# elvinlife/RadioSaber

Measured on AMD Instinct MI355X. Metric: scheduled TTIs/sec (and us/TTI) at 20 slices x 500 UEs x 25 RBGs; HBM GB/s, higher is better.
Workload: dtype f64

## Files before the change

### include/radiosaber_hip.h

```cpp
#ifndef RADIOSABER_HIP_H_
#define RADIOSABER_HIP_H_

#include <stddef.h>
#include <stdint.h>

#ifdef __cplusplus
extern "C" {
#endif

#define RS_ABI_VERSION 11

enum {
  RS_OK = 0,
  RS_ERR_INVALID = -1,
  RS_ERR_NO_DEVICE = -2,
  RS_ERR_HIP = -3,
  RS_ERR_STATE = -4,
  RS_ERR_RANGE = -5
};

enum {
  RS_SCHED_PF = 1,
  RS_SCHED_NVS = 7,
  RS_SCHED_SEQUENTIAL = 8,
  RS_SCHED_MAXCELL = 9,
  RS_SCHED_NVS_NONGREEDY = 11,
  RS_SCHED_UPPERBOUND = 10,
  RS_SCHED_SUBOPT = 101,
  RS_SCHED_VOGEL = 103
};

#define RS_MAX_SLICES 64
#define RS_MAX_RBGS 64
#define RS_MAX_USERS 1024

typedef struct rs_config {
  int32_t n_slices;
  int32_t n_users;
  int32_t n_rbgs;
  int32_t rbg_size;
  int32_t sched;
  int32_t device;
  const double* slice_weight;
  const int32_t* algo_alpha;
  const int32_t* algo_beta;
  const int32_t* algo_epsilon;
  const int32_t* algo_psi;
  const int32_t* user_to_slice;
  void* stream;
  int32_t synthetic_exp;
  int32_t link_tables;
} rs_config;

enum { RS_LINK_DEFAULT = 0, RS_LINK_HOST_LIBM = 1, RS_LINK_PINNED_GLIBC_2_35 = 2 };

const char* rs_last_error(void);
int rs_abi_version(void);
int rs_device_count(void);

int rs_link_tables(double eff[16], double kbps[16], double eesm_e[16], double eesm_x[16]);
int rs_link_tables_pinned(double eff[16], double kbps[16], double eesm_e[16], double eesm_x[16]);
int rs_link_tables_compare(char* msg, size_t msglen);

int rs_get_rbg_size(int nb_rbs);
int rs_dl_prbs_for_bandwidth(double bw_mhz);

typedef struct rs_ctx rs_ctx;

rs_ctx* rs_create(const rs_config* cfg);
rs_ctx* rs_create_checked(const rs_config* cfg, int abi_version, size_t cfg_size);
#define RS_CREATE(cfg) rs_create_checked((cfg), RS_ABI_VERSION, sizeof(rs_config))
void rs_destroy(rs_ctx* ctx);

typedef struct rs_tti_in {
  int32_t n_users;
  const int32_t* user_id;
  const uint8_t* cqi;
  const double* avg_rate;
  int32_t rand0, rand1;
  const uint8_t* cqi_prb;
  const double* hol_delay;
  const uint8_t* prio_has_data;
  const int32_t* rand_draws;
  const int32_t* required_rbs;
  const int32_t* data_to_transmit;
  uint64_t cqi_epoch;
} rs_tti_in;

typedef struct rs_tti_out {
  int32_t* target_rbs;
  int32_t* quota_rbgs;
  int32_t* rbg_to_user;
  int32_t* user_nprb;
  int32_t* user_final_cqi;
  int32_t* user_mcs;
  int32_t* user_tbs_bits;
  int32_t* upper_rbg;
  int32_t* upper_user;
} rs_tti_out;

int rs_schedule_tti(rs_ctx* ctx, const rs_tti_in* in, rs_tti_out* out);
int rs_ctx_specialize(rs_ctx* ctx);
int rs_ctx_jit_status(rs_ctx* ctx, char* msg, size_t msglen);
int rs_jit_selfcheck_dropin(int n_slices, int n_users, int n_rbgs, int rbg_size, int threads, int sched, char* err, size_t errlen);
int rs_get_slice_offset(rs_ctx* ctx, double* offset );
int rs_set_slice_offset(rs_ctx* ctx, const double* offset );

#define RS_GROUP_MAX_CELLS 1024
typedef struct rs_group rs_group;
rs_group* rs_group_create(const rs_config* cfg, int32_t n_cells);
rs_group* rs_group_create_checked(const rs_config* cfg, int32_t n_cells, int abi_version, size_t cfg_size);
#define RS_GROUP_CREATE(cfg, n_cells) rs_group_create_checked((cfg), (n_cells), RS_ABI_VERSION, sizeof(rs_config))
void rs_group_destroy(rs_group* g);
int rs_group_schedule_tti(rs_group* g, int32_t n, const int32_t* cell_ids, const rs_tti_in* in , rs_tti_out* out );
int rs_group_get_slice_offset(rs_group* g, int32_t cell, double* offset );
// ... 163 lines not shown
```

### radiosaber_amd/__init__.py

```python
from . import toolchain as _toolchain

_toolchain.prefer_system_compiler()

from .api import (
    RS_SCHED_MAXCELL, RS_SCHED_NVS, RS_SCHED_PF, RS_SCHED_NVS_NONGREEDY, RS_SCHED_SEQUENTIAL, RS_SCHED_UPPERBOUND, RS_SCHED_VOGEL, RS_SCHED_SUBOPT,
    BEARER_BACKLOG, BEARER_NONE, BEARER_QUEUE, FULL_PACKET, TRACE_CQI_HISTOGRAM, frames_to_bursts, internet_flow_arrivals,
    BatchScheduler, GroupScheduler, RadioSaberError, SliceConfig, TtiResult, TtiScheduler, device_count, device_source_hash, dl_prbs_for_bandwidth, get_rbg_size, hbm_copy_probe, jit_selfcheck, lds_bytes_per_cell,
    jit_cache_file, jit_cache_stats, jit_cache_warm, jit_compiler_identity, lib, link_tables_compare,
    RS_LINK_DEFAULT, RS_LINK_HOST_LIBM, RS_LINK_PINNED_GLIBC_2_35,
    link_tables, load_trace_dir, read_trace_mapping, read_ue_trace,
)

__all__ = ["RS_SCHED_PF", "RS_SCHED_NVS", "RS_SCHED_SEQUENTIAL", "RS_SCHED_MAXCELL", "RS_SCHED_VOGEL", "RS_SCHED_SUBOPT", "RS_SCHED_UPPERBOUND", "RS_SCHED_NVS_NONGREEDY", "SliceConfig",
           "TtiScheduler", "GroupScheduler", "TtiResult", "BatchScheduler", "RadioSaberError", "device_count", "lib",
           "link_tables", "jit_selfcheck", "device_source_hash", "TRACE_CQI_HISTOGRAM", "read_trace_mapping", "read_ue_trace",
           "load_trace_dir", "hbm_copy_probe", "lds_bytes_per_cell", "get_rbg_size", "dl_prbs_for_bandwidth", "internet_flow_arrivals", "frames_to_bursts",
           "BEARER_NONE", "BEARER_BACKLOG", "BEARER_QUEUE", "FULL_PACKET", "jit_cache_file", "jit_cache_stats", "jit_cache_warm",
           "jit_compiler_identity", "link_tables_compare", "RS_LINK_DEFAULT", "RS_LINK_HOST_LIBM", "RS_LINK_PINNED_GLIBC_2_35"]
```

### radiosaber_amd/api.py

```python
import ctypes as C
import json
import os
from dataclasses import dataclass, field
from pathlib import Path
from typing import List, Optional, Sequence

import numpy as np

RS_SCHED_SUBOPT = 101
RS_SCHED_PF, RS_SCHED_NVS, RS_SCHED_SEQUENTIAL, RS_SCHED_MAXCELL, RS_SCHED_UPPERBOUND, RS_SCHED_NVS_NONGREEDY, RS_SCHED_VOGEL = \
    1, 7, 8, 9, 10, 11, 103

TRACE_CQI_HISTOGRAM = (152600, 56656, 270880, 2088792, 3509504, 1595568, 4145392, 5295816, 1903424,
                       6890232, 4770864, 2842552, 3579624, 96000, 1227696)

_PKG = Path(__file__).resolve().parent
_LIB_PATH = Path(os.environ.get("RS_HIP_LIB", _PKG / "libradiosaber_hip.so"))


class RadioSaberError(RuntimeError):
    def __init__(self, code, msg):
        super().__init__(f"radiosaber_hip error {code}: {msg}")
        self.code = code

# ... 15 lines not shown


RS_LINK_DEFAULT, RS_LINK_HOST_LIBM, RS_LINK_PINNED_GLIBC_2_35 = 0, 1, 2

RS_ABI_VERSION = 11


class _TtiIn(C.Structure):
    _fields_ = [("n_users", C.c_int32), ("user_id", C.POINTER(C.c_int32)),
                ("cqi", C.POINTER(C.c_uint8)), ("avg_rate", C.POINTER(C.c_double)),
                ("rand0", C.c_int32), ("rand1", C.c_int32), ("cqi_prb", C.POINTER(C.c_uint8)),
                ("hol_delay", C.POINTER(C.c_double)), ("prio_has_data", C.POINTER(C.c_uint8)),
                ("rand_draws", C.POINTER(C.c_int32)),
                ("required_rbs", C.POINTER(C.c_int32)), ("data_to_transmit", C.POINTER(C.c_int32)), ("cqi_epoch", C.c_uint64)]


class _TtiOut(C.Structure):
    _fields_ = [("target_rbs", C.POINTER(C.c_int32)), ("quota_rbgs", C.POINTER(C.c_int32)),
                ("rbg_to_user", C.POINTER(C.c_int32)), ("user_nprb", C.POINTER(C.c_int32)),
                ("user_final_cqi", C.POINTER(C.c_int32)), ("user_mcs", C.POINTER(C.c_int32)),
                ("user_tbs_bits", C.POINTER(C.c_int32)),
                ("upper_rbg", C.POINTER(C.c_int32)), ("upper_user", C.POINTER(C.c_int32))]


class _BatchLog(C.Structure):
    _fields_ = [("rbg_to_user", C.POINTER(C.c_int16)), ("tbs_bits", C.POINTER(C.c_int32)),
                ("quota", C.POINTER(C.c_int16)), ("target", C.POINTER(C.c_int16)), ("uinfo", C.POINTER(C.c_int32)),
                ("slice_keys", C.POINTER(C.c_uint32))]


class _BatchBearerLog(C.Structure):
    _fields_ = [("bytes", C.POINTER(C.c_int32)), ("hol_delay", C.POINTER(C.c_double))]


ABI_SYMBOLS = [
    "rs_last_error", "rs_abi_version", "rs_device_count", "rs_link_tables",
    "rs_create", "rs_destroy", "rs_schedule_tti", "rs_get_slice_offset", "rs_set_slice_offset",
    "rs_batch_create", "rs_batch_destroy", "rs_batch_seed", "rs_batch_upload_cqi_epochs",
    "rs_batch_synthesize_cqi", "rs_batch_download_cqi_epochs", "rs_batch_set_trace",
    "rs_batch_run", "rs_batch_run_async", "rs_batch_sync", "rs_batch_run_logged",
    "rs_batch_run_timed", "rs_batch_read_state", "rs_batch_slice_bytes_device",
    "rs_batch_slice_bytes", "rs_jit_selfcheck", "rs_jit_selfcheck_queue", "rs_batch_debug_stamps", "rs_batch_ttis_done", "rs_batch_stream", "rs_batch_kernel_name",
    "rs_trace_read_mapping", "rs_trace_read_ue_log", "rs_trace_load_dir", "rs_hbm_copy_probe", "rs_lds_bytes_per_cell",
    "rs_get_rbg_size", "rs_dl_prbs_for_bandwidth", "rs_batch_synthesize_cqi_at", "rs_batch_run_logged_ex",
    "rs_batch_read_clock", "rs_batch_jit_status", "rs_batch_prepare_launch",
    "rs_batch_upload_cqi_epochs_prb", "rs_batch_set_trace_prb",
    "rs_batch_set_bearers", "rs_batch_set_arrivals", "rs_batch_read_bearer_state", "rs_internet_flow_arrivals",
    "rs_device_source_hash",
    "rs_create_checked", "rs_batch_create_checked", "rs_jit_selfcheck_untuned", "rs_batch_write_state",
    "rs_ctx_specialize", "rs_jit_selfcheck_dropin",
    "rs_batch_debug_heap_sorts", "rs_ctx_debug_heap_sorts",
    "rs_jit_cache_stats", "rs_jit_cache_file", "rs_jit_cache_warm", "rs_batch_autotune_report", "rs_batch_debug_clocks",
    "rs_batch_checkpoint_bytes", "rs_batch_checkpoint_save", "rs_batch_checkpoint_load",
    "rs_link_tables_pinned", "rs_link_tables_compare", "rs_ctx_jit_status", "rs_jit_compiler_identity",
    "rs_batch_flow_record", "rs_batch_run_logged_bearers",
    "rs_group_create", "rs_group_create_checked", "rs_group_destroy", "rs_group_schedule_tti",
    "rs_group_get_slice_offset", "rs_group_set_slice_offset", "rs_group_launch_count", "rs_group_kernel_name",
    "rs_group_image_stats", "rs_group_specialize", "rs_group_jit_status", "rs_jit_selfcheck_group",
    "rs_group_set_avg", "rs_group_get_avg", "rs_group_set_pending", "rs_group_schedule_tti_at", "rs_group_run_at",
    "rs_group_specialize_resident", "rs_group_resident_jit_status", "rs_jit_selfcheck_group_resident",
    "rs_group_set_bearers", "rs_group_get_bearers", "rs_group_schedule_tti_queued",
    "rs_group_specialize_queued", "rs_group_queued_jit_status", "rs_jit_selfcheck_group_queued",
    "rs_group_set_counters", "rs_group_get_counters", "rs_group_schedule_tti_counted",
    "rs_group_set_flows", "rs_group_get_flows", "rs_group_schedule_tti_flows",
    "rs_group_specialize_counted", "rs_group_counted_jit_status", "rs_jit_selfcheck_group_counted",
    "rs_group_specialize_flows", "rs_group_flows_jit_status", "rs_jit_selfcheck_group_flows",
    "rs_group_specialize_run", "rs_group_run_jit_status", "rs_jit_selfcheck_group_run",
]

_lib = None


def lib():
    global _lib
    if _lib is not None:
        return _lib
    if not _LIB_PATH.exists():
        raise RadioSaberError(-100, f"{_LIB_PATH} is missing: run `python -m radiosaber_amd.build` "
                                    "(there is no CPU fallback)")
    L = C.CDLL(str(_LIB_PATH))
    L.rs_last_error.restype = C.c_char_p
    L.rs_link_tables.argtypes = [C.POINTER(C.c_double)] * 4
    L.rs_link_tables_pinned.argtypes = [C.POINTER(C.c_double)] * 4
    L.rs_link_tables_compare.argtypes = [C.c_char_p, C.c_size_t]
    L.rs_ctx_jit_status.argtypes = [C.c_void_p, C.c_char_p, C.c_size_t]
    L.rs_jit_compiler_identity.restype = C.c_char_p
    L.rs_jit_compiler_identity.argtypes = []
    L.rs_create.restype = C.c_void_p
    L.rs_create.argtypes = [C.POINTER(_Config)]
    L.rs_destroy.argtypes = [C.c_void_p]
    L.rs_schedule_tti.argtypes = [C.c_void_p, C.POINTER(_TtiIn), C.POINTER(_TtiOut)]
    L.rs_get_slice_offset.argtypes = [C.c_void_p, C.POINTER(C.c_double)]
    L.rs_set_slice_offset.argtypes = [C.c_void_p, C.POINTER(C.c_double)]
    L.rs_group_create.restype = C.c_void_p
    L.rs_group_create.argtypes = [C.POINTER(_Config), C.c_int32]
    L.rs_group_create_checked.restype = C.c_void_p
    L.rs_group_create_checked.argtypes = [C.POINTER(_Config), C.c_int32, C.c_int, C.c_size_t]
    L.rs_group_destroy.argtypes = [C.c_void_p]
    L.rs_group_schedule_tti.argtypes = [C.c_void_p, C.c_int32, C.POINTER(C.c_int32), C.POINTER(_TtiIn), C.POINTER(_TtiOut)]
    L.rs_group_get_slice_offset.argtypes = [C.c_void_p, C.c_int32, C.POINTER(C.c_double)]
    L.rs_group_set_slice_offset.argtypes = [C.c_void_p, C.c_int32, C.POINTER(C.c_double)]
    L.rs_group_launch_count.restype = C.c_int64
    L.rs_group_launch_count.argtypes = [C.c_void_p]
    L.rs_group_image_stats.argtypes = [C.c_void_p, C.POINTER(C.c_int64)]
    L.rs_group_kernel_name.restype = C.c_char_p
    L.rs_group_kernel_name.argtypes = [C.c_void_p]
    L.rs_group_specialize.argtypes = [C.c_void_p]
    L.rs_group_set_avg.argtypes = [C.c_void_p, C.c_int32, C.POINTER(C.c_double), C.c_double]
    L.rs_group_get_avg.argtypes = [C.c_void_p, C.c_int32, C.POINTER(C.c_double), C.POINTER(C.c_int32), C.POINTER(C.c_double)]
    L.rs_group_set_pending.argtypes = [C.c_void_p, C.c_int32, C.POINTER(C.c_int32)]
    L.rs_group_schedule_tti_at.argtypes = [C.c_void_p, C.c_int32, C.POINTER(C.c_int32), C.POINTER(_TtiIn), C.POINTER(_TtiOut), C.POINTER(C.c_double)]
    L.rs_group_run_at.argtypes = [C.c_void_p, C.c_int32, C.POINTER(C.c_int32), C.POINTER(_TtiIn), C.c_int32, C.POINTER(C.c_double),
                                  C.POINTER(C.c_int32), C.POINTER(_TtiOut)]
    L.rs_group_set_bearers.argtypes = [C.c_void_p, C.c_int32, C.POINTER(C.c_uint8), C.POINTER(C.c_double), C.c_double]
    L.rs_group_get_bearers.argtypes = [C.c_void_p, C.c_int32, C.POINTER(C.c_double), C.POINTER(C.c_int32), C.POINTER(C.c_double)]
    L.rs_group_schedule_tti_queued.argtypes = [C.c_void_p, C.c_int32, C.POINTER(C.c_int32), C.POINTER(_TtiIn), C.POINTER(_TtiOut),
                                               C.POINTER(C.c_double), C.POINTER(C.POINTER(C.c_int32))]
    L.rs_group_jit_status.argtypes = [C.c_void_p, C.c_char_p, C.c_size_t]
    L.rs_jit_selfcheck_group.argtypes = [C.c_int] * 6 + [C.c_char_p, C.c_size_t]
    L.rs_group_specialize_resident.argtypes = [C.c_void_p]
    L.rs_group_resident_jit_status.argtypes = [C.c_void_p, C.c_char_p, C.c_size_t]
    L.rs_jit_selfcheck_group_resident.argtypes = [C.c_int] * 6 + [C.c_char_p, C.c_size_t]
    L.rs_group_set_counters.argtypes = [C.c_void_p, C.c_int32, C.POINTER(C.c_int64), C.POINTER(C.c_int64)]
    L.rs_group_get_counters.argtypes = [C.c_void_p, C.c_int32, C.POINTER(C.c_int64), C.POINTER(C.c_int64)]
    L.rs_group_schedule_tti_counted.argtypes = [C.c_void_p, C.c_int32, C.POINTER(C.c_int32), C.POINTER(_TtiIn), C.POINTER(_TtiOut),
                                                C.POINTER(C.c_double), C.POINTER(C.POINTER(C.c_int32)), C.POINTER(C.POINTER(C.c_int32))]
    L.rs_group_set_flows.argtypes = [C.c_void_p, C.c_int32, C.POINTER(C.c_uint8), C.POINTER(C.c_double), C.c_double, C.POINTER(C.c_int64),
                                     C.POINTER(C.c_int64)]
    L.rs_group_get_flows.argtypes = [C.c_void_p, C.c_int32, C.POINTER(C.c_double), C.POINTER(C.c_int32), C.POINTER(C.c_double),
                                     C.POINTER(C.c_int64), C.POINTER(C.c_int64)]
    L.rs_group_schedule_tti_flows.argtypes = [C.c_void_p, C.c_int32, C.POINTER(C.c_int32), C.POINTER(_TtiIn), C.POINTER(_TtiOut),
                                              C.POINTER(C.c_double), C.POINTER(C.POINTER(C.c_uint8))]
    L.rs_group_specialize_queued.argtypes = [C.c_void_p]
    L.rs_group_queued_jit_status.argtypes = [C.c_void_p, C.c_char_p, C.c_size_t]
    L.rs_jit_selfcheck_group_queued.argtypes = [C.c_int] * 6 + [C.c_char_p, C.c_size_t]
    L.rs_group_specialize_counted.argtypes = [C.c_void_p]
# ... 102 lines not shown
                  group=False, resident=False, queued=False, counted=False, flows=False, run=False):
    _jit_flags(False, False, group, resident, queued, counted, flows, run)
    buf = C.create_string_buffer(4096)
    fn = lib().rs_jit_selfcheck_queue if queues else (lib().rs_jit_selfcheck_untuned if untuned else lib().rs_jit_selfcheck)
    if dropin:
        fn = lib().rs_jit_selfcheck_dropin
    if group:
        fn = lib().rs_jit_selfcheck_group_resident if resident else lib().rs_jit_selfcheck_group
        if queued:
            fn = lib().rs_jit_selfcheck_group_queued
        if counted:
            fn = lib().rs_jit_selfcheck_group_counted
        if flows:
            fn = lib().rs_jit_selfcheck_group_flows
        if run:
            fn = lib().rs_jit_selfcheck_group_run
    n = fn(n_slices, n_users, n_rbgs, rbg_size, threads, sched, buf, 4096)
    if n < 0:
        raise RadioSaberError(n, buf.value.decode(errors="replace"))
    return n


def jit_cache_stats():
    out = (C.c_longlong * 4)()
    lib().rs_jit_cache_stats(out)
    return dict(zip(("hits", "misses", "stores", "rejected"), (int(x) for x in out)))


def _jit_flags(lean, streamed, group, resident, queued=False, counted=False, flows=False, run=False):
    if run and not (group and resident):
        raise ValueError("run=True needs group=True and resident=True: the run kernel is the resident form's")
    if run and (queued or counted or flows):
        raise ValueError("run=True excludes queued=True, counted=True and flows=True: only the resident form has a run")
    if counted and not group:
        raise ValueError("counted=True needs group=True: only a group has a counted kernel")
    if flows and not group:
        raise ValueError("flows=True needs group=True: only a group has a flows kernel")
    if counted and resident:
        raise ValueError("resident=True and counted=True exclude each other: two forms of a group's kernel")
    if flows and (resident or queued or counted):
        raise ValueError("flows=True excludes resident=True, queued=True and counted=True: a form of a group's kernel of its own")
    if counted:
        queued = True
    if resident and not group:
        raise ValueError("resident=True needs group=True: only a group has a resident kernel")
    if queued and not group:
        raise ValueError("queued=True needs group=True: only a group has a queued kernel")
    if queued and resident:
        raise ValueError("resident=True and queued=True exclude each other: two forms of a group's kernel")
    return (4 if lean else 0) | (2 if streamed else 0) | (8 if group else 0) | (16 if resident else 0) | (32 if queued else 0) | \
        (64 if counted else 0) | (128 if flows else 0) | (256 if run else 0)


def jit_cache_file(n_slices, n_users, n_rbgs, rbg_size, threads=512, sched=RS_SCHED_MAXCELL, lean=False, streamed=False, group=False,
                   resident=False, queued=False, counted=False, flows=False, run=False):
    buf = C.create_string_buffer(4096)
    lib().rs_jit_cache_file(n_slices, n_users, n_rbgs, rbg_size, threads, sched, _jit_flags(lean, streamed, group, resident, queued, counted, flows, run),
                            buf, 4096)
    return buf.value.decode()


def jit_cache_warm(n_slices, n_users, n_rbgs, rbg_size, threads=512, sched=RS_SCHED_MAXCELL, lean=False, streamed=False, group=False,
                   resident=False, queued=False, counted=False, flows=False, run=False):
    buf = C.create_string_buffer(4096)
    n = lib().rs_jit_cache_warm(n_slices, n_users, n_rbgs, rbg_size, threads, sched, _jit_flags(lean, streamed, group, resident, queued, counted, flows, run),
                                buf, 4096)
    if n < 0:
        raise RadioSaberError(n, buf.value.decode(errors="replace"))
    return n


def device_count():
    return lib().rs_device_count()


def device_source_hash():
    return lib().rs_device_source_hash().decode()


def get_rbg_size(nb_rbs):
    return _count(lib().rs_get_rbg_size(nb_rbs))


def dl_prbs_for_bandwidth(bw_mhz):
    return lib().rs_dl_prbs_for_bandwidth(float(bw_mhz))


BEARER_NONE, BEARER_BACKLOG, BEARER_QUEUE = 0, 1, 2
FULL_PACKET = 1495


def internet_flow_arrivals(rate_mbps, start_time, stop_time, size_seed, max_bursts=1 << 16):
    t = np.zeros(max_bursts, np.float64)
    nf = np.zeros(max_bursts, np.int32)
    la = np.zeros(max_bursts, np.int32)
    n = _count(lib().rs_internet_flow_arrivals(rate_mbps, start_time, stop_time, size_seed, max_bursts, _p(t, C.c_double),
                                               _p(nf, C.c_int32), _p(la, C.c_int32)))
    return t[:n].copy(), nf[:n].copy(), la[:n].copy()


def frames_to_bursts(times, frame_bytes, mtu=1490):
    fb = np.asarray(frame_bytes, np.int64)
    rem = fb % mtu
    return (np.ascontiguousarray(times, np.float64), (fb // mtu).astype(np.int32),
            np.where(rem > 0, rem + (FULL_PACKET - mtu), 0).astype(np.int32))


def lds_bytes_per_cell(n_slices, n_users, n_rbgs, sched=RS_SCHED_MAXCELL, threads=512):
    return _count(lib().rs_lds_bytes_per_cell(n_slices, n_users, n_rbgs, sched, threads))


def hbm_copy_probe(device=0, nbytes=1 << 30, iters=10):
    g = C.c_double(0)
    _check(lib().rs_hbm_copy_probe(device, nbytes, iters, C.byref(g)))
    return g.value


def link_tables(pinned=False):
    out = [np.zeros(16, np.float64) for _ in range(4)]
    _check((lib().rs_link_tables_pinned if pinned else lib().rs_link_tables)(*[_p(a, C.c_double) for a in out]))
    return dict(zip(("eff", "kbps", "eesm_e", "eesm_x"), out))


def link_tables_compare():
    buf = C.create_string_buffer(4096)
    return _count(lib().rs_link_tables_compare(buf, 4096)), buf.value.decode(errors="replace")


def jit_compiler_identity():
    return lib().rs_jit_compiler_identity().decode()


def read_trace_mapping(path, max_entries=4096):
    out = np.zeros(max_entries, dtype=np.int32)
    n = _count(lib().rs_trace_read_mapping(os.fsencode(str(path)), _p(out, C.c_int32), max_entries))
    if n > max_entries:
        raise RadioSaberError(-1, f"{path}: {n} entries, max_entries={max_entries}")
    return out[:n].copy()


def read_ue_trace(path, nb_rbs=512, rbg_size=8, n_rows=475, per_prb=False):
    R = nb_rbs // rbg_size
    rbg = np.zeros((n_rows, R), dtype=np.uint8)
    prb = np.zeros((n_rows, nb_rbs), dtype=np.uint8) if per_prb else None
    rc = _count(lib().rs_trace_read_ue_log(os.fsencode(str(path)), n_rows, nb_rbs, rbg_size, _p(rbg, C.c_uint8),
                                           _p(prb, C.c_uint8) if per_prb else None))
    return (prb if per_prb else rbg), rc


def load_trace_dir(directory, n_traces=158, nb_rbs=512, rbg_size=8, n_rows=475):
    R = nb_rbs // rbg_size
    out = np.zeros((n_traces, n_rows, R), dtype=np.uint8)
    rc = _count(lib().rs_trace_load_dir(os.fsencode(str(directory)), n_traces, n_rows, nb_rbs, rbg_size,
                                        _p(out, C.c_uint8)))
    return out, rc


@dataclass
class SliceConfig:
    ues_per_slice: List[int]
    weight: List[float] = field(default_factory=list)
    algo_alpha: List[int] = field(default_factory=list)
    algo_beta: List[int] = field(default_factory=list)
    algo_epsilon: List[int] = field(default_factory=list)
    algo_psi: List[int] = field(default_factory=list)
    traffic: List[dict] = field(default_factory=list)

    def __post_init__(self):
        S = len(self.ues_per_slice)
        if not self.weight:
            self.weight = [1.0 / S] * S
        for name, default in (("algo_alpha", 0), ("algo_beta", 0), ("algo_epsilon", 1), ("algo_psi", 1)):
            if not getattr(self, name):
                setattr(self, name, [default] * S)
# ... 618 lines not shown
        _check(lib().rs_batch_set_arrivals(self._h, _p(off, C.c_int64), _p(t_all, C.c_double), _p(nf_all, C.c_int32),
                                           _p(la_all, C.c_int32)))
        self._burst_slots = {key: (int(off[(key[0] * self.U + key[1]) * 2 + key[2]]), len(v[0])) for key, v in bursts.items()}
        self._n_bursts = total

    def flow_record(self):
        if not hasattr(self, "_burst_slots"):
            raise RadioSaberError(-4, "flow_record() before set_arrivals()")
        tti = np.zeros(max(self._n_bursts, 1), np.int32)
        tm = np.zeros(max(self._n_bursts, 1), np.float64)
        _check(lib().rs_batch_flow_record(self._h, _p(tti, C.c_int32), _p(tm, C.c_double)))
        return {key: (tti[i:i + n].copy(), tm[i:i + n].copy()) for key, (i, n) in self._burst_slots.items()}

    def bearer_state(self):
        shp = (self.n_cells, self.U, 2)
        avg, cb, cr = np.zeros(shp, np.float64), np.zeros(shp, np.int64), np.zeros(shp, np.int64)
        qb, qp = np.zeros(shp, np.int32), np.zeros(shp, np.int32)
        _check(lib().rs_batch_read_bearer_state(self._h, _p(avg, C.c_double), _p(cb, C.c_int64), _p(cr, C.c_int64),
                                                _p(qb, C.c_int32), _p(qp, C.c_int32)))
        return {"avg_rate": avg, "cum_bytes": cb, "cum_rbs": cr, "queue_bytes": qb, "queue_packets": qp}

    def clock(self):
        t = np.zeros(self.n_cells, np.float64)
        lu = np.zeros(self.n_cells, np.float64)
        _check(lib().rs_batch_read_clock(self._h, _p(t, C.c_double), _p(lu, C.c_double)))
        return t, lu

    def prepare_launch(self, n_ttis):
        _check(lib().rs_batch_prepare_launch(self._h, int(n_ttis)))

    def checkpoint(self):
        n = _count(lib().rs_batch_checkpoint_bytes(self._h))
        buf = C.create_string_buffer(n)
        _check(lib().rs_batch_checkpoint_save(self._h, buf, n))
        return buf.raw

    def restore(self, blob):
        _check(lib().rs_batch_checkpoint_load(self._h, blob, len(blob)))

    def debug_clocks(self):
        mhz = np.zeros(self.n_cells, np.float64)
        ms = np.zeros(self.n_cells, np.float64)
        _check(lib().rs_batch_debug_clocks(self._h, _p(mhz, C.c_double), _p(ms, C.c_double)))
        return mhz, ms

    def autotune_report(self):
        buf = C.create_string_buffer(1024)
        n = lib().rs_batch_autotune_report(self._h, buf, 1024)
        return n, buf.value.decode(errors="replace")

    def jit_status(self):
        if not getattr(self, "_h", None):
            raise RadioSaberError(-4, "jit_status() of a closed batch")
        buf = C.create_string_buffer(512)
        rc = lib().rs_batch_jit_status(self._h, buf, 512)
        return rc, buf.value.decode(errors="replace")

    def slice_bytes(self):
        out = np.zeros(self.S, np.uint64)
        _check(lib().rs_batch_slice_bytes(self._h, _p(out, C.c_uint64)))
        return out

    def slice_bytes_into(self, device_ptr):
        _check(lib().rs_batch_slice_bytes_device(self._h, C.c_void_p(device_ptr)))

    def heap_sorts(self):
        out = np.zeros((self.n_cells, 3), np.int64)
        _check(lib().rs_batch_debug_heap_sorts(self._h, _p(out, C.c_int64)))
        return out

    def debug_stamps(self, cell=0):
        out = np.zeros(20, np.uint64)
        _check(lib().rs_batch_debug_stamps(self._h, cell, _p(out, C.c_uint64)))
        return out

    @property
    def ttis_done(self):
        return lib().rs_batch_ttis_done(self._h)

    @property
    def stream(self):
        return lib().rs_batch_stream(self._h)

    @property
    def kernel_name(self):
        return lib().rs_batch_kernel_name(self._h).decode()
```

### radiosaber_amd/csrc/rs_api.cpp

```cpp
#include <hip/hip_runtime_api.h>

#include <atomic>
#include <chrono>
#include <cmath>
#include <cstdarg>
#include <cstdio>
#include <cstdlib>
#include <cstring>
#include <new>
#include <random>
#include <fstream>
#include <vector>

#include "../../include/radiosaber_hip.h"
#include "rs_amc_tables.inc"
#include "rs_link_pinned.inc"
#include "rs_device.h"

extern "C" hipError_t rs_launch_cells(const RsLaunch* p, int threads, hipStream_t stream);
extern "C" hipError_t rs_prepare_kernels(int max_lds_bytes);
struct RsJitKernel;
extern "C" RsJitKernel* rs_jit_get(int device, int S, int U, int R, int G, int NT, int sched, int qmode, int win, char* err, size_t errlen,
                                   int flags,
                                   const char* variant = nullptr);
extern "C" int rs_jit_is_untuned(const RsJitKernel* k);
extern "C" int rs_jit_is_verified(const RsJitKernel* k);
extern "C" int rs_jit_was_loaded(const RsJitKernel* k);
extern "C" void rs_jit_mark_verified(RsJitKernel* k);
extern "C" void rs_jit_reject(RsJitKernel* k);
extern "C" hipError_t rs_jit_launch(RsJitKernel* k, const RsLaunch* p, hipStream_t stream);
extern "C" hipError_t rs_launch_synth(uint8_t* epochs, int64_t grid_stride, int n_cells, int n_epochs, int U, int R, int Upad,
                                      uint64_t seed, int64_t first_cell, const uint32_t* cdf16, hipStream_t stream);
extern "C" hipError_t rs_launch_copy_probe(const void* src, void* dst, size_t bytes, hipStream_t stream);
extern "C" hipError_t rs_launch_slice_bytes(const int64_t* cum_bytes, const uint8_t* user_slice, int n_cells, int U,
                                            int S, unsigned long long* d_out, hipStream_t stream);

namespace {

thread_local char g_err[512] = "";

int fail(int code, const char* fmt, ...) {
  va_list ap;
  va_start(ap, fmt);
  vsnprintf(g_err, sizeof g_err, fmt, ap);
  va_end(ap);
  return code;
}

#define HIP_TRY(expr)                                                                          \
  do {                                                                                         \
    hipError_t e__ = (expr);                                                                   \
    if (e__ != hipSuccess) return fail(RS_ERR_HIP, "%s: %s", #expr, hipGetErrorString(e__));   \
  } while (0)

struct ScratchBuffers {
// ... 125 lines not shown
int rs_link_tables_compare(char* msg, size_t msglen) {
  double eff[16], kbps[16], e[16], x[16];
  if (msg && msglen) msg[0] = 0;
  const int rc = rs_link_tables(eff, kbps, e, x);
  if (rc) return rc;
  int diff = 0;
  std::string text;
  char line[160];
  for (int c = 1; c <= 15; c++)
    if (to_bits(e[c]) != to_bits(kPinnedE[c - 1])) {
      diff++;
      snprintf(line, sizeof line, "E[%d] host %a pinned %a; ", c, e[c], kPinnedE[c - 1]);
      text += line;
    }
  for (int k = 1; k <= 13; k++)
    if (to_bits(x[k]) != to_bits(kPinnedX[k - 1])) {
      diff++;
      snprintf(line, sizeof line, "X[%d] host %a pinned %a; ", k, x[k], kPinnedX[k - 1]);
      text += line;
    }
  if (msg && msglen) snprintf(msg, msglen, "%s", text.c_str());
  return diff;
}

int rs_link_tables(double eff[16], double kbps[16], double eesm_e[16], double eesm_x[16]) {
  eff[0] = kbps[0] = eesm_e[0] = eesm_x[0] = 0;
  for (int c = 1; c <= 15; c++) {
    int bits = kTbs[0][kMcsToItbs[kCqiToMcs[c - 1]]];
    double e = (bits / 0.001) / 180000.;
    eff[c] = e;
    kbps[c] = e * 180000 / 1000;
    double s = pow(10, kSinrForCqi[c - 1] / 10);
    double beta = 1;
    eesm_e[c] = exp(-s / beta);
  }
  eesm_x[14] = eesm_x[15] = 0;
  for (int k = 1; k <= 13; k++) {
    const double thr = kSinrForCqi[k];
    uint64_t lo = 1, hi = to_bits(1.0) - 1;
    if (!(eesm_db_of_mean(from_bits(lo)) >= thr)) return fail(RS_ERR_INVALID, "EESM threshold %d unreachable", k);
    while (hi - lo > 1) {
      uint64_t mid = lo + (hi - lo) / 2;
      if (eesm_db_of_mean(from_bits(mid)) >= thr) lo = mid; else hi = mid;
    }
    if (eesm_db_of_mean(from_bits(hi)) >= thr) lo = hi;
    for (int d = 1; d <= 4096; d++) {
      if (!(eesm_db_of_mean(from_bits(lo - d)) >= thr) || (eesm_db_of_mean(from_bits(lo + d)) >= thr))
        return fail(RS_ERR_INVALID, "host libm not monotone around EESM threshold %d (offset %d ulp)", k, d);
    }
    eesm_x[k] = from_bits(lo);
  }
  for (int k = 2; k <= 13; k++)
    if (!(eesm_x[k] < eesm_x[k - 1])) return fail(RS_ERR_INVALID, "EESM thresholds not decreasing at %d", k);
  return RS_OK;
}

}


struct rs_batch {
  rs_batch_config cfg;
  std::vector<double> weight;
  std::vector<int32_t> eps, psi, u2s, alpha, beta;
  bool any_alpha = false;
  bool synthetic = false;
  bool gen_exp = false;
  double* d_gen_num = nullptr;
  int32_t *d_alpha = nullptr, *d_beta = nullptr;
  int S, U, R, G, sched, n_cells, threads;
  bool direct = false;
  hipStream_t stream = nullptr;
  bool own_stream = false;
  RsTables* d_tab = nullptr;
  double* d_weight = nullptr;
  int32_t *d_eps = nullptr, *d_psi = nullptr;
  uint8_t* d_user_slice = nullptr;
  int32_t* d_tbs_eff = nullptr;
  double* d_avg = nullptr;
  int32_t* d_tx = nullptr;
  int64_t *d_cumb = nullptr, *d_cumr = nullptr;
  double* d_sstate = nullptr;
  RsCellScalars* d_scal = nullptr;
  uint8_t* d_epochs = nullptr;
  int64_t grid_stride = 0;
  int32_t n_epochs = 0;
  uint8_t* d_trace = nullptr;
  int32_t n_traces = 0, n_rows = 0, row_mod = 0;
  int32_t* d_user_trace = nullptr;
  uint8_t *d_epochs_prb = nullptr, *d_trace_prb = nullptr;
  int64_t grid_stride_prb = 0;
  int32_t cqi_mode = RS_CQI_NONE;
  int32_t* d_err = nullptr;
  unsigned long long* d_slice_bytes = nullptr;
  unsigned long long* d_stamps = nullptr;
  bool queues = false;
  int qmode = 2;
  uint8_t* d_bearer_kind = nullptr;
  int64_t* d_arr_off = nullptr;
  double* d_arr_time = nullptr;
  int32_t *d_arr_nfull = nullptr, *d_arr_last = nullptr;
  int32_t* d_qi = nullptr;
  double* d_bavg = nullptr;
  int64_t* d_bcum = nullptr;
  uint8_t* d_qflags = nullptr;
  double* d_qhol = nullptr;
  int32_t* d_flow_tti = nullptr;
  double* d_flow_time = nullptr;
  size_t n_bursts = 0;
  RsJitKernel* jit = nullptr;
  RsJitKernel* jit_lean = nullptr;
  bool jit_lean_tried = false;
  bool autotuned = false;
  bool selfchecked = false;
  bool selfchecked_general = false, selfchecked_lean = false;
  bool in_selfcheck = false;
  bool jit_rejected = false;
  char selfcheck_msg[160] = "";
  int autotune_n = 0;
  char autotune_msg[768] = "";
  unsigned long long* d_prio_sum = nullptr;
  bool jit_wanted = false;
  char jit_msg[512] = "";
  int64_t ttis_done = 0;
  RsLaunch base{};
};

namespace {

int validate(const rs_config* c, bool direct) {
  if (!c) return fail(RS_ERR_INVALID, "null config");
// ... 85 lines not shown
    b->stream = (hipStream_t)b->cfg.cell.stream;
  } else {
    HIP_TRY(hipStreamCreateWithFlags(&b->stream, hipStreamNonBlocking));
    b->own_stream = true;
  }
  RsTables t;
  memset(&t, 0, sizeof t);
  double eff[16];
  const int link = b->cfg.cell.link_tables != RS_LINK_DEFAULT ? b->cfg.cell.link_tables : (b->direct ? RS_LINK_HOST_LIBM : RS_LINK_PINNED_GLIBC_2_35);
  int rc = link == RS_LINK_PINNED_GLIBC_2_35 ? rs_link_tables_pinned(eff, t.kbps, t.eesm_e, t.eesm_x) : rs_link_tables(eff, t.kbps, t.eesm_e, t.eesm_x);
  if (rc) return rc;
  for (int c = 1; c <= 15; c++) {
    t.pfnum[c] = eff[c] * 180000.;
    t.eff[c] = eff[c];
    t.mcs_of_cqi[c] = kCqiToMcs[c - 1];
    t.itbs_of_cqi[c] = kMcsToItbs[kCqiToMcs[c - 1]];
    t.tbs1_of_cqi[c] = kTbs[0][kMcsToItbs[kCqiToMcs[c - 1]]];
    int rt = 1;
    while (rt <= 14 && kSinrForCqi[rt] <= kSinrForCqi[c - 1]) rt++;
    t.tbs1_syn[c] = kTbs[0][kMcsToItbs[kCqiToMcs[rt - 1]]];
  }
  for (int i = 0; i < 27; i++) t.tbs_row_m1[i] = i <= 23 ? kMcsToItbs[5 + i] : 0;
  HIP_TRY(hipMalloc(&b->d_tab, sizeof t));
  HIP_TRY(hipMemcpy(b->d_tab, &t, sizeof t, hipMemcpyHostToDevice));
  HIP_TRY(hipMalloc(&b->d_weight, 8 * S));
  HIP_TRY(hipMemcpy(b->d_weight, b->weight.data(), 8 * S, hipMemcpyHostToDevice));
  HIP_TRY(hipMalloc(&b->d_eps, 4 * S));
  HIP_TRY(hipMemcpy(b->d_eps, b->eps.data(), 4 * S, hipMemcpyHostToDevice));
  HIP_TRY(hipMalloc(&b->d_psi, 4 * S));
  HIP_TRY(hipMemcpy(b->d_psi, b->psi.data(), 4 * S, hipMemcpyHostToDevice));
  HIP_TRY(hipMalloc(&b->d_alpha, 4 * S));
  HIP_TRY(hipMemcpy(b->d_alpha, b->alpha.data(), 4 * S, hipMemcpyHostToDevice));
  HIP_TRY(hipMalloc(&b->d_beta, 4 * S));
  HIP_TRY(hipMemcpy(b->d_beta, b->beta.data(), 4 * S, hipMemcpyHostToDevice));
  std::vector<uint8_t> us(U);
  for (size_t u = 0; u < U; u++) us[u] = (uint8_t)b->u2s[u];
  HIP_TRY(hipMalloc(&b->d_user_slice, U));
  HIP_TRY(hipMemcpy(b->d_user_slice, us.data(), U, hipMemcpyHostToDevice));
  {
    std::vector<int32_t> te((size_t)(b->R + 1) * 27, 0);
    for (int n = 1; n <= b->R; n++)
      for (int i = 0; i < 27; i++) {
        const int nprb = n * b->G;
        int v;
        if (nprb <= 110) v = kTbs[nprb - 1][i];
        else v = 5 * kTbs[nprb / 5 - 1][i] + (nprb % 5 == 0 ? t.tbs_row_m1[i] : kTbs[nprb % 5 - 1][i]);
        te[(size_t)n * 27 + i] = v;
      }
    for (int32_t v : te)
      if (v / 8 > RS_MAX_BYTES_PER_TTI) return fail(RS_ERR_INVALID, "a transport block of %d bits does not fit the per-launch byte counters", v);
    std::vector<int32_t> te16((size_t)(b->R + 1) * 16, 0);
    for (int n = 0; n <= b->R; n++)
      for (int c = 0; c < 16; c++) te16[(size_t)n * 16 + c] = te[(size_t)n * 27 + t.itbs_of_cqi[c]];
    HIP_TRY(hipMalloc(&b->d_tbs_eff, 4 * te16.size()));
    HIP_TRY(hipMemcpy(b->d_tbs_eff, te16.data(), 4 * te16.size(), hipMemcpyHostToDevice));
  }
  if (b->gen_exp) {
    std::vector<double> gn((size_t)S * 16, 0.0);
    for (size_t s = 0; s < S; s++)
      for (int c = 1; c <= 15; c++) gn[s * 16 + c] = pow(t.kbps[c], b->eps[s]);
    HIP_TRY(hipMalloc(&b->d_gen_num, 8 * gn.size()));
    HIP_TRY(hipMemcpy(b->d_gen_num, gn.data(), 8 * gn.size(), hipMemcpyHostToDevice));
  }
  HIP_TRY(hipMalloc(&b->d_avg, 8 * cells * U));
  HIP_TRY(hipMalloc(&b->d_tx, 4 * cells * U));
  HIP_TRY(hipMalloc(&b->d_cumb, 8 * cells * U));
  HIP_TRY(hipMalloc(&b->d_cumr, 8 * cells * U));
  HIP_TRY(hipMalloc(&b->d_sstate, 8 * cells * S));
  HIP_TRY(hipMalloc(&b->d_scal, sizeof(RsCellScalars) * cells));
  HIP_TRY(hipMalloc(&b->d_err, 4));
  HIP_TRY(hipMalloc(&b->d_slice_bytes, 8 * 64));
  HIP_TRY(hipMemset(b->d_err, 0, 4));
#ifdef RS_STAMPS
  HIP_TRY(hipMalloc(&b->d_stamps, 8 * 20 * (size_t)b->n_cells));
  HIP_TRY(hipMemset(b->d_stamps, 0, 8 * 20 * (size_t)b->n_cells));
#endif
  std::vector<double> avg(cells * U, 100000.0);
  HIP_TRY(hipMemcpy(b->d_avg, avg.data(), 8 * cells * U, hipMemcpyHostToDevice));
  HIP_TRY(hipMemset(b->d_tx, 0, 4 * cells * U));
  HIP_TRY(hipMemset(b->d_cumb, 0, 8 * cells * U));
  HIP_TRY(hipMemset(b->d_cumr, 0, 8 * cells * U));
  HIP_TRY(hipMemset(b->d_sstate, 0, 8 * cells * S));
  rc = init_scalars(b, nullptr, nullptr);
  if (rc) return rc;

  RsLaunch& L = b->base;
  memset(&L, 0, sizeof L);
  L.S = b->S; L.U = b->U; L.R = b->R; L.G = b->G;
  L.sched = b->sched;
  L.n_cells = b->n_cells;
  L.refresh = b->cfg.cqi_refresh;
  L.epoch_wrap = b->cfg.cqi_epoch_wrap ? 1 : 0;
  L.phy_draws = b->cfg.phy_error_draws;
  L.tab = b->d_tab; L.weight = b->d_weight; L.eps = b->d_eps; L.psi = b->d_psi;
  L.alpha = b->d_alpha; L.beta = b->d_beta;
  L.user_slice = b->d_user_slice;
  L.tbs_eff = b->d_tbs_eff;
  L.synthetic = b->synthetic ? 1 : 0;
  L.avg = b->d_avg; L.tx_bytes = b->d_tx; L.cum_bytes = b->d_cumb; L.cum_rbs = b->d_cumr;
  L.slice_state = b->d_sstate; L.scal = b->d_scal; L.err = b->d_err; L.stamps = b->d_stamps;
  carve_lds(b, &L);
  if (L.lds_bytes > 160 * 1024) return fail(RS_ERR_INVALID, "cell needs %d B of LDS (> 160 KiB)", L.lds_bytes);
  {
    hipDeviceProp_t prop;
    int cus = 256;
    if (hipGetDeviceProperties(&prop, b->cfg.cell.device) == hipSuccess && prop.multiProcessorCount > 0) cus = prop.multiProcessorCount;
    int mode = (!b->direct && b->n_cells > cus) ? 2 : 0;
    if (const char* e = getenv("RS_PRIO_BALANCE")) mode = b->direct ? 0 : atoi(e);
    L.prio_round_cells = mode == 1 ? cus : 0;
    if (mode == 2) {
      HIP_TRY(hipMalloc(&b->d_prio_sum, 8));
      HIP_TRY(hipMemset(b->d_prio_sum, 0, 8));
      L.prio_sum = b->d_prio_sum;
    }
  }
  HIP_TRY(rs_prepare_kernels(160 * 1024));
  return RS_OK;
}

rs_batch* batch_new(const rs_batch_config* cfg, bool direct) {
  if (!cfg) { fail(RS_ERR_INVALID, "null config"); return nullptr; }
  if (validate(&cfg->cell, direct)) return nullptr;
  if (cfg->n_cells < 1) { fail(RS_ERR_INVALID, "n_cells %d < 1", cfg->n_cells); return nullptr; }
  if (!direct && cfg->cqi_refresh < 1) { fail(RS_ERR_INVALID, "cqi_refresh %d < 1", cfg->cqi_refresh); return nullptr; }
  if (cfg->first_tti < 0) { fail(RS_ERR_INVALID, "first_tti %d < 0", cfg->first_tti); return nullptr; }
  int threads = cfg->threads_per_cell;
  if (threads == 0) {
    hipDeviceProp_t prop;
    int cus = 256;
    if (hipGetDeviceProperties(&prop, cfg->cell.device) == hipSuccess && prop.multiProcessorCount > 0)
      cus = prop.multiProcessorCount;
    threads = (!direct && cfg->n_cells >= 4 * cus) ? 256 : 512;
  }
  int want_jit = cfg->jit;
  if (const char* e = getenv("RS_JIT")) want_jit = atoi(e);
  const int max_threads = (want_jit && !direct) ? 1024 : 512;
  if (threads % 64 || threads < 64 || threads > max_threads) {
    fail(RS_ERR_INVALID, "threads_per_cell %d (a multiple of 64 in 64..%d%s)", threads, max_threads,
         max_threads == 512 ? "; up to 1024 with jit = 1" : "");
    return nullptr;
  }
  if ((cfg->cqi_epoch_wrap | 1) != 1) { fail(RS_ERR_INVALID, "cqi_epoch_wrap %d is not 0 or 1", cfg->cqi_epoch_wrap); return nullptr; }
  if ((cfg->autotune | 1) != 1) { fail(RS_ERR_INVALID, "autotune %d is not 0 or 1", cfg->autotune); return nullptr; }
  if (cfg->selfcheck < -1 || cfg->selfcheck > 1) { fail(RS_ERR_INVALID, "selfcheck %d outside -1..1", cfg->selfcheck); return nullptr; }
  if (cfg->queue_state_lds < -1 || cfg->queue_state_lds > 1) { fail(RS_ERR_INVALID, "queue_state_lds %d outside -1..1", cfg->queue_state_lds); return nullptr; }
  if (cfg->cell.sched == RS_SCHED_UPPERBOUND) {
    const int N = cfg->cell.n_rbgs * cfg->cell.n_slices;
    if (cfg->threads_per_cell == 0)
      while (threads < 512 && N > 4 * threads) threads += 64;
    if (N > 4 * threads) {
      fail(RS_ERR_INVALID, "RS_SCHED_UPPERBOUND: n_rbgs * n_slices = %d exceeds 4 * threads_per_cell = %d", N, 4 * threads);
      return nullptr;
    }
  }
  int n = 0;
  if (hipGetDeviceCount(&n) != hipSuccess || n == 0) { fail(RS_ERR_NO_DEVICE, "no HIP device"); return nullptr; }
  if (cfg->cell.device < 0 || cfg->cell.device >= n) { fail(RS_ERR_NO_DEVICE, "device %d of %d", cfg->cell.device, n); return nullptr; }
  rs_batch* b = new (std::nothrow) rs_batch();
  if (!b) { fail(RS_ERR_INVALID, "out of memory"); return nullptr; }
  b->cfg = *cfg;
  const rs_config& c = cfg->cell;
  b->S = c.n_slices; b->U = c.n_users; b->R = c.n_rbgs; b->G = c.rbg_size; b->sched = c.sched;
  b->n_cells = cfg->n_cells;
  b->threads = threads;
  b->direct = direct;
  b->weight.assign(c.slice_weight, c.slice_weight + b->S);
  b->eps.assign(c.algo_epsilon, c.algo_epsilon + b->S);
  b->psi.assign(c.algo_psi, c.algo_psi + b->S);
  b->alpha.assign(c.algo_alpha, c.algo_alpha + b->S);
  b->beta.assign(b->S, 0);
  if (c.algo_beta) b->beta.assign(c.algo_beta, c.algo_beta + b->S);
  b->synthetic = c.synthetic_exp != 0;
  for (int s = 0; s < b->S; s++) b->any_alpha |= b->alpha[s] != 0;
  for (int s = 0; s < b->S; s++)
    b->gen_exp |= direct && c.sched != RS_SCHED_PF && c.sched != RS_SCHED_NVS_NONGREEDY && ((b->eps[s] | 1) != 1 || (b->psi[s] | 1) != 1);
  b->u2s.assign(c.user_to_slice, c.user_to_slice + b->U);
  b->cfg.cell.slice_weight = nullptr; b->cfg.cell.algo_alpha = nullptr; b->cfg.cell.algo_beta = nullptr;
  b->cfg.cell.algo_epsilon = nullptr; b->cfg.cell.algo_psi = nullptr; b->cfg.cell.user_to_slice = nullptr;
  b->jit_wanted = want_jit && !direct;
  if (batch_alloc(b)) { rs_batch_destroy(b); return nullptr; }
  if (want_jit && !direct) {
    b->jit_wanted = true;
    b->jit = rs_jit_get(b->cfg.cell.device, b->S, b->U, b->R, b->G, b->threads, b->sched, 0, slice_window(b), b->jit_msg, sizeof b->jit_msg,
                        b->cfg.cqi_refresh <= 4 ? 2 : 0);
    if (b->jit) snprintf(b->jit_msg, sizeof b->jit_msg, "%s", rs_jit_is_untuned(b->jit) ? "in use, built WITHOUT the -mllvm tuning options (hiprtc refused them): a few per cent slower" : "");
    else if (!b->jit_msg[0]) snprintf(b->jit_msg, sizeof b->jit_msg, "hiprtc build failed");
    if (!b->jit && b->threads > 512) {
      fail(RS_ERR_INVALID, "threads_per_cell %d needs the shape-specialised kernel, which could not be built: %s", b->threads, b->jit_msg);
      rs_batch_destroy(b);
      return nullptr;
    }
  }
  return b;
}

int check_device_err(rs_batch* b) {
  int e = 0;
  HIP_TRY(hipSetDevice(b->cfg.cell.device));
  HIP_TRY(hipMemcpy(&e, b->d_err, 4, hipMemcpyDeviceToHost));
  if (e) {
    HIP_TRY(hipMemset(b->d_err, 0, 4));
    return fail(RS_ERR_RANGE, e == RS_CQI_EPOCHS ? "ran past the last CQI epoch" : "trace row outside the uploaded rows");
  }
  return RS_OK;
}

RsJitKernel* lean_kernel(rs_batch* b, int n_ttis, bool logged) {
  if (!b->jit || b->direct || logged) return nullptr;
  const char* const e_min = getenv("RS_JIT_LEAN_MIN_TTIS");
  const char* const e_on = getenv("RS_JIT_LEAN");
  const int lean_min = e_min ? atoi(e_min) : 256;
  if (e_on && atoi(e_on) == 0) return nullptr;
  if (n_ttis < lean_min || b->cqi_mode != RS_CQI_EPOCHS || b->d_epochs_prb || b->cfg.phy_error_draws || b->synthetic) return nullptr;
  if (!b->jit_lean_tried) {
    b->jit_lean_tried = true;
    char msg[512] = "";
    b->jit_lean = rs_jit_get(b->cfg.cell.device, b->S, b->U, b->R, b->G, b->threads, b->sched, b->queues ? b->qmode : 0, slice_window(b), msg,
                             sizeof msg, (b->cfg.cqi_refresh <= 4 ? 2 : 0) | 4);
    if (!b->jit_lean) snprintf(b->jit_msg, sizeof b->jit_msg, "lean build unavailable, the general build serves every launch (%.400s)", msg);
  }
  return b->jit_lean;
}

int launch(rs_batch* b, int n_ttis, int16_t* d_map, int16_t* d_quota, int16_t* d_target, int32_t* d_tbs, int32_t* d_uinfo,
           uint32_t* d_keys = nullptr, int32_t* d_bbytes = nullptr, double* d_bhol = nullptr);

struct StatePart { void* p; size_t n; };
std::vector<StatePart> state_parts(rs_batch* b) {
  const size_t cells = b->n_cells, U = b->U, S = b->S, n2 = cells * 2 * U;
  std::vector<StatePart> v = {{b->d_avg, 8 * cells * U}, {b->d_tx, 4 * cells * U}, {b->d_cumb, 8 * cells * U}, {b->d_cumr, 8 * cells * U},
                              {b->d_sstate, 8 * cells * S}, {b->d_scal, sizeof(RsCellScalars) * cells}};
  if (b->queues) {
    v.push_back({b->d_qi, 4 * 7 * n2});
    v.push_back({b->d_bavg, 8 * n2});
    v.push_back({b->d_bcum, 8 * 2 * n2});
    v.push_back({b->d_qflags, cells * U});
    v.push_back({b->d_qhol, 8 * cells * U});
  }
  return v;
}

struct StateParts {
  std::vector<StatePart> parts;
  size_t total = 0;
  explicit StateParts(rs_batch* b, bool with_record = false) : parts(state_parts(b)) {
    if (with_record && b->queues && b->d_flow_tti) {
      parts.push_back({b->d_flow_tti, 4 * b->n_bursts});
      parts.push_back({b->d_flow_time, 8 * b->n_bursts});
    }
    for (const StatePart& q : parts) total += (q.n + 255) & ~(size_t)255;
  }
  hipError_t copy(rs_batch* b, void* snapshot, bool save) const {
    size_t off = 0;
    for (const StatePart& q : parts) {
      void* snap = (char*)snapshot + off;
      const hipError_t e = hipMemcpyAsync(save ? snap : q.p, save ? q.p : snap, q.n, hipMemcpyDeviceToDevice, b->stream);
      if (e != hipSuccess) return e;
      off += (q.n + 255) & ~(size_t)255;
    }
    return hipSuccess;
  }
};

struct StateDigest {
  unsigned long long part[14] = {0, 0, 0, 0, 0, 0, 0, 0, 0, 0, 0, 0, 0, 0};
  bool operator==(const StateDigest& o) const { return memcmp(part, o.part, sizeof part) == 0; }
  bool operator!=(const StateDigest& o) const { return !(*this == o); }
  std::string diff(const StateDigest& o) const {
    static const char* const names[14] = {"PF averages", "cumulative bytes", "cumulative RBs", "slice state", "pending grants", "simulated time",
                                          "last EWMA update", "TTIs done", "users served in the last TTI", "rand() ring / CQI-report state",
                                          "bearers' queues", "bearers' PF averages", "bearers' cumulative counters", "flow completion record"};
// ... 40 lines not shown
    const size_t n2 = cells * 2 * U;
    const StatePart q[3] = {{b->d_qi, 4 * 7 * n2}, {b->d_bavg, 8 * n2}, {b->d_bcum, 8 * 2 * n2}};
    for (int i = 0; i < 3; i++) {
      std::vector<unsigned char> hq(q[i].n);
      HIP_TRY(hipMemcpy(hq.data(), q[i].p, q[i].n, hipMemcpyDeviceToHost));
      out->part[10 + i] = fnv(hq.data(), q[i].n);
    }
    if (b->d_flow_tti) {
      std::vector<unsigned char> hr(12 * b->n_bursts);
      HIP_TRY(hipMemcpy(hr.data(), b->d_flow_tti, 4 * b->n_bursts, hipMemcpyDeviceToHost));
      HIP_TRY(hipMemcpy(hr.data() + 4 * b->n_bursts, b->d_flow_time, 8 * b->n_bursts, hipMemcpyDeviceToHost));
      out->part[13] = fnv(hr.data(), hr.size());
    }
  }
  return RS_OK;
}

int autotune(rs_batch* b, int n_ttis) {
  if (b->autotuned || !b->cfg.autotune) return RS_OK;
  if (!lean_kernel(b, n_ttis, false)) return RS_OK;
  b->autotuned = true;
  const int sched = b->sched;
  if (b->queues || b->direct || !(sched == 8 || sched == 9 || sched == 101 || sched == 103)) return RS_OK;
  const int win = slice_window(b);
  std::vector<std::string> cand = {""};
  const bool ilp_by_rule = sched == 9 || (sched == 8 && (b->R > 32 || win > 0));
  cand.push_back(ilp_by_rule ? "ss=default" : "ss=iterative-ilp");
  cand.push_back(b->R > 32 ? "-DRS_NO_SPEC" : "-DRS_NO_HOLD");
  if (sched == 9) cand.push_back("-DRS_P3_BLOCK=8");
  const StateParts sp(b);
  ScratchBuffers scratch;
  ScratchEvents events;
  void* snapshot = nullptr;
  RsJitKernel* const k_default = b->jit_lean;
  const int64_t done0 = b->ttis_done;
  struct Restore {
    rs_batch* b; RsJitKernel* k; int64_t done;
    ~Restore() { b->jit_lean = k; b->ttis_done = done; }
  } restore{b, k_default, done0};
  HIP_TRY(scratch.alloc(&snapshot, sp.total));
  HIP_TRY(events.create(2));
  const hipEvent_t e0 = events.ev[0], e1 = events.ev[1];
  const int trial = n_ttis < 512 ? n_ttis : 512;
  RsJitKernel* best = k_default;
  float best_ms = 0, default_ms = 0;
  StateDigest default_digest;
  int rc = RS_OK;
  HIP_TRY(sp.copy(b, snapshot, true));
  std::string report;
  for (size_t i = 0; i < cand.size() && rc == RS_OK; i++) {
    char msg[512] = "";
    RsJitKernel* k = i == 0 ? k_default
                            : rs_jit_get(b->cfg.cell.device, b->S, b->U, b->R, b->G, b->threads, sched, 0, win, msg, sizeof msg,
                                         (b->cfg.cqi_refresh <= 4 ? 2 : 0) | 4, cand[i].c_str());
    if (!k) { report += cand[i] + ": not built; "; continue; }
    b->jit_lean = k;
    float ms = 0;
    for (int rep = 0; rep < 3 && rc == RS_OK; rep++) {
      if (sp.copy(b, snapshot, false) != hipSuccess || hipEventRecord(e0, b->stream) != hipSuccess) { rc = fail(RS_ERR_HIP, "autotune: state restore failed"); break; }
      rc = launch(b, trial, nullptr, nullptr, nullptr, nullptr, nullptr, nullptr);
      if (rc) break;
      float t = 0;
      if (hipEventRecord(e1, b->stream) != hipSuccess || hipEventSynchronize(e1) != hipSuccess || hipEventElapsedTime(&t, e0, e1) != hipSuccess) {
        rc = fail(RS_ERR_HIP, "autotune: timing failed");
        break;
      }
      if (rep == 1 || (rep == 2 && t < ms)) ms = t;
    }
    if (rc) break;
    StateDigest digest;
    rc = state_digest(b, &digest);
    if (rc) break;
    if (i == 0) default_digest = digest;
    char line[320];
    if (digest != default_digest) {
      snprintf(line, sizeof line, "%s: %.3f ms, REJECTED: its state after the trial differs from the rule table's build (%s); ", cand[i].c_str(), ms,
               digest.diff(default_digest).c_str());
      report += line;
      rs_jit_reject(k);
      continue;
    }
    if (i > 0 && rs_jit_is_verified(k_default)) rs_jit_mark_verified(k);
    snprintf(line, sizeof line, "%s: %.3f ms; ", i == 0 ? "rule table" : cand[i].c_str(), ms);
    report += line;
    b->autotune_n++;
    if (i == 0) { best = k; best_ms = default_ms = ms; }
    else if (ms < best_ms && ms < 0.99f * default_ms) { best = k; best_ms = ms; }
  }
  const hipError_t back = sp.copy(b, snapshot, false);
  const hipError_t sync = hipStreamSynchronize(b->stream);
  if (back != hipSuccess || sync != hipSuccess) return fail(RS_ERR_HIP, "autotune: the cell state could not be put back");
  if (rc) return rc;
  rc = check_device_err(b);
  if (rc) return rc;
  restore.k = best;
  snprintf(b->autotune_msg, sizeof b->autotune_msg, "autotune over %d TTIs: %skept %s", trial, report.c_str(),
           best == k_default ? "the rule table's build" : "the fastest");
  return RS_OK;
}

enum { kCheckNever = 0, kCheckUnmarked = 1, kCheckAll = 2 };
int selfcheck_policy(const rs_batch* b) {
  if (b->cfg.selfcheck > 0) return kCheckAll;
  if (b->cfg.selfcheck < 0) return kCheckNever;
  const char* e = getenv("RS_JIT_SELFCHECK");
  if (e && e[0] == '0') return kCheckNever;
  if (e && e[0] == '2') return kCheckAll;
// ... 727 lines not shown
        else if (!want_packed && h.packed_tx) w &= RS_TX_BYTES_MASK;
      }
      HIP_TRY(hipMemcpy(q.p, tx.data(), q.n, hipMemcpyHostToDevice));
    } else {
      HIP_TRY(hipMemcpy(q.p, in, q.n, hipMemcpyHostToDevice));
    }
    in += q.n;
  }
  b->ttis_done = h.ttis_done;
  return RS_OK;
}

int rs_batch_debug_clocks(rs_batch* b, double* shader_mhz, double* kernel_ms) {
  if (!b) return fail(RS_ERR_INVALID, "null batch");
  HIP_TRY(hipSetDevice(b->cfg.cell.device));
  HIP_TRY(hipStreamSynchronize(b->stream));
  std::vector<RsCellScalars> sc(b->n_cells);
  HIP_TRY(hipMemcpy(sc.data(), b->d_scal, sizeof(RsCellScalars) * b->n_cells, hipMemcpyDeviceToHost));
  for (int c = 0; c < b->n_cells; c++) {
    const double real = (double)(sc[c].real_end - sc[c].real_begin), clk = (double)(sc[c].clk_end - sc[c].clk_begin);
    if (shader_mhz) shader_mhz[c] = real > 0 ? clk / real * 100.0 : 0.0;
    if (kernel_ms) kernel_ms[c] = real / 1e5;
  }
  return RS_OK;
}

int rs_batch_autotune_report(rs_batch* b, char* msg, size_t msglen) {
  if (!b) return fail(RS_ERR_INVALID, "null batch");
  if (msg && msglen) snprintf(msg, msglen, "%s", b->autotune_msg);
  return b->autotune_n;
}

int rs_batch_prepare_launch(rs_batch* b, int32_t n_ttis) {
  if (!b || n_ttis < 1) return fail(RS_ERR_INVALID, "bad argument");
  if (b->cqi_mode == RS_CQI_NONE) return fail(RS_ERR_STATE, "no CQI source set");
  HIP_TRY(hipSetDevice(b->cfg.cell.device));
  (void)lean_kernel(b, n_ttis > RS_MAX_TTIS_PER_LAUNCH ? RS_MAX_TTIS_PER_LAUNCH : n_ttis, false);
  if (!b->selfchecked) {
    const int rc = selfcheck(b, n_ttis > RS_MAX_TTIS_PER_LAUNCH ? RS_MAX_TTIS_PER_LAUNCH : n_ttis, false);
    if (rc) return rc;
  }
  if (b->cfg.autotune && !b->autotuned) {
    const int rc = autotune(b, n_ttis > RS_MAX_TTIS_PER_LAUNCH ? RS_MAX_TTIS_PER_LAUNCH : n_ttis);
    if (rc) return rc;
  }
  return RS_OK;
}

int rs_batch_jit_status(rs_batch* b, char* msg, size_t msglen) {
  if (!b) return fail(RS_ERR_INVALID, "null batch");
  if (msg && msglen) snprintf(msg, msglen, "%s", b->jit_msg);
  if (b->jit_rejected) return -2;
  if (msg && msglen && b->jit && !b->jit_msg[0] && b->selfcheck_msg[0]) snprintf(msg, msglen, "%s", b->selfcheck_msg);
  return b->jit ? 1 : (b->jit_wanted ? -1 : 0);
}

int rs_batch_slice_bytes_device(rs_batch* b, uint64_t* d_out) {
  if (!b || !d_out) return fail(RS_ERR_INVALID, "null argument");
  HIP_TRY(hipSetDevice(b->cfg.cell.device));
  HIP_TRY(rs_launch_slice_bytes(b->d_cumb, b->d_user_slice, b->n_cells, b->U, b->S, (unsigned long long*)d_out, b->stream));
  return RS_OK;
}

int rs_batch_slice_bytes(rs_batch* b, uint64_t* h_out) {
  if (!b || !h_out) return fail(RS_ERR_INVALID, "null argument");
  int rc = rs_batch_slice_bytes_device(b, (uint64_t*)b->d_slice_bytes);
  if (rc) return rc;
  HIP_TRY(hipStreamSynchronize(b->stream));
  HIP_TRY(hipMemcpy(h_out, b->d_slice_bytes, 8 * b->S, hipMemcpyDeviceToHost));
  return RS_OK;
}

int rs_batch_debug_stamps(rs_batch* b, int32_t cell, uint64_t* out20) {
  if (!b || !out20 || cell < 0 || cell >= b->n_cells) return fail(RS_ERR_INVALID, "bad argument");
  if (!b->d_stamps) return fail(RS_ERR_STATE, "not a diagnostic (-DRS_STAMPS) build");
  HIP_TRY(hipStreamSynchronize(b->stream));
  HIP_TRY(hipMemcpy(out20, b->d_stamps + (size_t)cell * 20, 8 * 20, hipMemcpyDeviceToHost));
  return RS_OK;
}

int64_t rs_batch_ttis_done(rs_batch* b) { return b ? b->ttis_done : -1; }
void* rs_batch_stream(rs_batch* b) { return b ? (void*)b->stream : nullptr; }
const char* rs_batch_kernel_name(rs_batch* b) {
  if (!b) return "";
  if (b->jit) return "rs_cell_kernel_jit";
  switch (b->sched) {
    case 1: return "rs_cell_kernel<1, 0, false>";
    case 7: return "rs_cell_kernel<7, 0, false>";
    case 8: return "rs_cell_kernel<8, 0, false>";
    case RS_SCHED_SUBOPT: return "rs_cell_kernel<101, 0, false>";
    case RS_SCHED_VOGEL: return "rs_cell_kernel<103, 0, false>";
    case RS_SCHED_NVS_NONGREEDY: return "rs_cell_kernel<11, 0, false>";
    case RS_SCHED_UPPERBOUND: {
      const int ept = (b->R * b->S + b->threads - 1) / b->threads;
      return ept <= 1 ? "rs_cell_kernel<10, 1, false>" : ept <= 2 ? "rs_cell_kernel<10, 2, false>" : ept <= 3 ? "rs_cell_kernel<10, 3, false>" : "rs_cell_kernel<10, 4, false>";
    }
    default: {
      const int ept = (b->R * b->S + b->threads - 1) / b->threads;
      return ept <= 1 ? "rs_cell_kernel<9, 1, false>" : ept <= 2 ? "rs_cell_kernel<9, 2, false>" : ept <= 3 ? "rs_cell_kernel<9, 3, false>" : ept <= 4 ? "rs_cell_kernel<9, 4, false>" : "rs_cell_kernel<9, 0, false>";
    }
  }
}

}


// ... 2040 lines not shown
```

### radiosaber_amd/csrc/rs_device.h

```cpp
#ifndef RS_DEVICE_H_
#define RS_DEVICE_H_

#ifndef __HIPCC_RTC__
#include <stdint.h>
#elif !defined(RS_RTC_STDINT)
#define RS_RTC_STDINT
typedef signed char int8_t;
typedef unsigned char uint8_t;
typedef short int16_t;
typedef unsigned short uint16_t;
typedef int int32_t;
typedef unsigned int uint32_t;
typedef long long int64_t;
typedef unsigned long long uint64_t;
typedef unsigned long size_t;
#endif

#define RS_WAVE 64
#define RS_TX_BYTES_MASK 0xFFFFF
#define RS_TX_NPRB_SHIFT 20
#define RS_TX_NPRB_MASK 0x3FF
#define RS_TX_COUNTED (1 << 30)
#define RS_FULL_PACKET 1495
#define RS_MAX_TTIS_PER_LAUNCH 32768
#define RS_MAX_BYTES_PER_TTI 65535
#define RS_PF_SEG 32

#define RS_MAX_SEGS 256
struct RsSpecFlags {
  int32_t ctr_p1, ctr_p3, greedy_done, n_fix;
};
#define RS_FIX_CAP 960
struct RsMisc {
  unsigned long long maskA[64], maskB[64];
  int32_t seg_begin[68];
  int32_t target[64];
  int32_t quota[64];
  int32_t n_level[48];
  uint16_t hist[64 * 16];
  int32_t mcs_of_cqi[16];
  int32_t tbs1_of_cqi[16];
  int32_t served;
  int32_t nvs_slice;
  int32_t pad[2];
  float ones16[16];
  double eff16[16];
  uint8_t eps_psi[64];
  int32_t rcp_off[64];
  RsSpecFlags spec[2];
  int32_t grid_free;
  int32_t heap_sorts[3];
  int32_t prio_boost;
  int32_t pad3[3];
};

struct RsCarve {
  int Upad, n_seg, n_items, ept, nvs_seg;
  int off_avgk, off_rcp, off_tab, off_slice, off_tx, off_misc, off_tbs, off_elems, off_sorted, off_items,
      off_sortx, off_cqi, off_queue, off_qstate, q_lds, lds_bytes;
};
constexpr int rs_round_up(int x, int a) { return (x + a - 1) / a * a; }
constexpr int rs_upad_of(int U) {
  int k = (U + 7) / 8;
  return 8 * ((k & 1) ? k : k + 1);
}
#ifndef RS_UMAP_SCRATCH_BYTES
#define RS_UMAP_SCRATCH_BYTES 272
#endif
#define RS_NVS_SAMPLES 300
#define RS_NVS_DRAW_BYTES 8192
#define RS_NVS_BATCH 64
constexpr int rs_nvs_pack(int batch, int draw_bytes, int val_bytes) { return batch | ((draw_bytes >> 10) << 8) | ((val_bytes >> 4) << 16); }
constexpr int rs_nvs_batch_of(int seg) { return seg & 0xff; }
constexpr int rs_nvs_draw_of(int seg) { return ((seg >> 8) & 0xff) << 10; }
constexpr int rs_nvs_val_of(int seg) { return (seg >> 16) << 4; }
constexpr int rs_nvs_key_bytes(int n, int R) { return 32 * n + 32 * n * ((R + 3) / 4); }
constexpr int rs_nvs_val_bytes(int U, int R, int win, int choice) {
  const int w = win > 0 && win < U ? win : U;
  const int keyed = w <= 64 ? rs_nvs_key_bytes(w, R) : 0;
  const int longest = keyed > 32 * w ? keyed : 32 * w;
  return rs_round_up(choice == 1 ? longest : (choice == 2 ? 32 * U : (longest > 32 * U ? longest : 32 * U)), 16);
}
constexpr int rs_nvs_scratch_bytes(int U, int R, int seg) {
  return rs_nvs_val_of(seg) + rs_nvs_draw_of(seg) + 2 * rs_nvs_batch_of(seg) * ((R + 3) / 4 * 4) + 128 + (U + 15) / 16 * 16;
}
#define RS_QSTATE_BYTES_PER_USER 156
#define RS_LDS_LIMIT (160 * 1024)
constexpr int rs_sort_cuts_bytes(int N) { return rs_round_up(4 * (N / 16 + 2), 16); }
constexpr int rs_sort_ranks_bytes(int N) { return ((N + 63) / 64) * 64 > 1024 ? 2 * 64 * ((N + 63) / 64) : 0; }
constexpr RsCarve rs_carve_with(int S, int U, int R, int sched, int threads, int nvs_seg, int queue = 0) {
  RsCarve c{};
  c.Upad = rs_upad_of(U);
  c.nvs_seg = nvs_seg;
  c.n_seg = sched == 1 ? (U + RS_PF_SEG - 1) / RS_PF_SEG
                     : (sched == 7 ? (nvs_seg ? (U + nvs_seg - 1) / nvs_seg + 1 : 1) : (sched == 11 ? 1 : S));
  c.n_items = R * c.n_seg;
  c.ept = (R * S + threads - 1) / threads;
  const bool pf_like = sched == 1 || (sched == 7 && nvs_seg != 0);
  int off = 8 * U;
  c.off_avgk = off; off += 8 * U;
  c.off_rcp = off; off += rs_round_up(4 * (c.Upad + 16 * S) + 2 * U, 16);
  c.off_tab = off; off += 8 * 48 + 64;
  c.off_slice = off; off += 8 * 128;
  c.off_tx = off; off += rs_round_up(4 * U, 16);
  c.off_misc = off; off += rs_round_up((int)sizeof(RsMisc), 16);
  c.off_tbs = off; off += rs_round_up(4 * 16 * (R + 1), 16);
  c.off_elems = off; off += sched == 11 ? 0 : rs_round_up(pf_like ? 8 * c.n_items : 4 * R * S, 16);
  c.off_sorted = off; off += (sched == 1 || sched == 7 || sched == 11) ? 0 : rs_round_up(4 * R * S, 16);
  const bool spec = sched == 8 || sched == 9 || sched == 101 || sched == 103;
  c.off_items = off; off += rs_round_up((spec ? 4 : 2) * c.n_items, 16);
  c.off_sortx = off; off += (sched == 9 || sched == 10) ? rs_round_up(c.ept <= 4 ? rs_sort_cuts_bytes(R * S) + rs_sort_ranks_bytes(R * S) : 8 * R * S, 16)
                                                           : (sched == 11 ? rs_round_up(rs_nvs_scratch_bytes(U, R, nvs_seg), 16) : (sched == 101 ? RS_UMAP_SCRATCH_BYTES : 0));
  c.off_cqi = off; off += rs_round_up(c.Upad * R, 16);
  c.off_queue = off; off += (queue && (sched == 1 || sched == 7)) ? rs_round_up(18 * U, 16) : 0;
  c.off_qstate = off;
  c.q_lds = (queue == 2 && off + rs_round_up(RS_QSTATE_BYTES_PER_USER * U, 16) <= RS_LDS_LIMIT) ? 1 : 0;
  off += c.q_lds ? rs_round_up(RS_QSTATE_BYTES_PER_USER * U, 16) : 0;
  c.lds_bytes = off;
  return c;
}
#ifndef RS_NVS_WHOLE_SLICE
#define RS_NVS_WHOLE_SLICE 64
#endif
#ifndef RS_NVS_WHOLE_SLICE_BUILTIN
#define RS_NVS_WHOLE_SLICE_BUILTIN 32
#endif
constexpr RsCarve rs_carve(int S, int U, int R, int sched, int threads, int queue = 0, int win = 0, int nvs_whole = RS_NVS_WHOLE_SLICE) {
  if (queue) return rs_carve_with(S, U, R, sched, threads, 0, queue);
  const bool nvs_long = sched == 7 && (win > 0 ? win > nvs_whole : U > nvs_whole * S);
  if (nvs_long) {
    for (int seg = 8; seg <= 16; seg *= 2) {
      const RsCarve c = rs_carve_with(S, U, R, sched, threads, seg);
      if (c.lds_bytes <= 80 * 1024) return c;
    }
  }
  if (nvs_long) return rs_carve_with(S, U, R, sched, threads, 32);
  if (sched == 11) {
    for (int choice = 0; choice <= 2; ++choice) {
      const int val = rs_nvs_val_bytes(U, R, win, choice);
      const RsCarve c0 = rs_carve_with(S, U, R, sched, threads, rs_nvs_pack(64, RS_NVS_DRAW_BYTES, val));
      if (c0.lds_bytes <= 80 * 1024) return c0;
      const RsCarve c1 = rs_carve_with(S, U, R, sched, threads, rs_nvs_pack(64, RS_NVS_DRAW_BYTES / 2, val));
      if (c1.lds_bytes <= 80 * 1024) return c1;
      const RsCarve c2 = rs_carve_with(S, U, R, sched, threads, rs_nvs_pack(32, RS_NVS_DRAW_BYTES / 2, val));
      if (c2.lds_bytes <= 80 * 1024) return c2;
    }
    return rs_carve_with(S, U, R, sched, threads, rs_nvs_pack(64, RS_NVS_DRAW_BYTES, rs_nvs_val_bytes(U, R, win, 0)));
  }
  return rs_carve_with(S, U, R, sched, threads, 0);
}

struct RsTables {
  double kbps[16];
  double pfnum[16];
  double eff[16];
  double eesm_e[16];
  double eesm_x[16];
  int32_t mcs_of_cqi[16];
  int32_t itbs_of_cqi[16];
  int32_t tbs_row_m1[28];
  int32_t tbs1_of_cqi[16];
  int32_t tbs1_syn[16];
};

struct RsCellScalars {
  double t;
  double last_update;
  int64_t last_sent;
  int32_t reported;
  int32_t served_prev;
  int64_t n_done;
  int32_t rng_f, rng_b;
  uint32_t rng_r[32];
  int32_t cqi_row;
  int32_t pad_;
  int64_t heap_sorts[3];
  uint64_t clk_begin, clk_end, real_begin, real_end;
};

enum { RS_CQI_NONE = 0, RS_CQI_EPOCHS = 1, RS_CQI_TRACE = 2 };

struct RsLaunch {
  int32_t S, U, R, G;
  int32_t Upad;
  int32_t nvs_seg;
  int32_t sched;
  int32_t n_cells, n_ttis;
  int32_t refresh, phy_draws;
  int32_t epoch_wrap;
  int32_t direct;
  int32_t rand0, rand1;
  const RsTables* tab;
  const double* weight;
  const int32_t* eps;
  const int32_t* psi;
  const uint8_t* user_slice;
  const uint8_t* prb_cqi;
  int32_t queue_mode;
  const int32_t* alpha;
  const int32_t* beta;
  const double* hol;
  const uint8_t* prio;
  const uint8_t* bearer_kind;
// ... 97 lines not shown
```

### radiosaber_amd/csrc/rs_jit.cpp

```cpp
#include <hip/hip_runtime_api.h>
#include <hip/hiprtc.h>

#include <dlfcn.h>
#include <fcntl.h>
#include <sys/stat.h>
#include <unistd.h>

#include <atomic>
#include <cerrno>
#include <cstdio>
#include <cstdlib>
#include <cstring>
#include <map>
#include <mutex>
#include <string>
#include <vector>

#include "rs_device.h"
#include "rs_jit_sources.inc"

struct RsJitKernel {
  hipModule_t mod = nullptr;
  hipFunction_t fn = nullptr;
  int threads = 0;
  int lds_bytes = 0, q_lds = 0;
  bool untuned = false;
  bool from_cache = false, verified = false, rejected = false;
  std::string cache_file, key_text, what;
};

namespace {
std::mutex g_mu;
std::map<std::string, RsJitKernel*> g_cache;
}

static int rs_jit_waves_per_simd(int NT, int lds_bytes) {
  if (NT <= 512) return 4;
  const int cells = 2 * lds_bytes <= RS_LDS_LIMIT ? 2 : 1;
  const int wpe = (cells * (NT / 64) + 3) / 4;
  return wpe < 4 ? 4 : (wpe > 8 ? 8 : wpe);
}

static std::vector<std::string> rs_jit_options(int S, int U, int R, int G, int NT, int sched, int qmode, int win, bool tuned, bool direct,
                                               bool streamed, bool lean, const char* variant = nullptr, bool group = false, bool resident = false,
                                               bool queued = false, bool counted = false, bool flows = false, bool run = false) {
  const RsCarve cv = rs_carve(S, U, R, sched, NT, qmode, win);
  std::vector<std::string> o = {"--offload-arch=gfx950", "-O3", "-std=c++17", "-ffp-contract=off", "-DRS_JIT_BUILD=1",
                                "-DRS_JIT_S=" + std::to_string(S), "-DRS_JIT_U=" + std::to_string(U),
                                "-DRS_JIT_R=" + std::to_string(R), "-DRS_JIT_G=" + std::to_string(G),
                                "-DRS_JIT_NT=" + std::to_string(NT), "-DRS_JIT_SCHED=" + std::to_string(sched),
                                "-DRS_JIT_CARVEQ=" + std::to_string(qmode), "-DRS_JIT_DIRECT=" + std::to_string(direct ? 1 : 0),
                                "-DRS_JIT_WPE=" + std::to_string(rs_jit_waves_per_simd(NT, cv.lds_bytes)),
                                "-DRS_JIT_WIN=" + std::to_string(win)};
  const int ept = (R * S + NT - 1) / NT;
  o.push_back("-DRS_P3_BLOCK=" + std::to_string((sched != 9 && sched != 10) ? 32 : ((ept <= 1 || (!qmode && !direct)) ? 16 : 8)));
  if (sched == 9 && !qmode && !direct && R <= 32) o.push_back("-DRS_P3_BLOCK_TOP=8");
  if ((sched == 8 || sched == 101 || sched == 103) && !qmode && !direct && R <= 32 && (win > 32 || streamed)) o.push_back("-DRS_P3_BLOCK_TOP=8");
  if (streamed && !direct) o.push_back("-DRS_JIT_STREAMED=1");
  if (lean) o.push_back("-DRS_JIT_LEAN=1");
  if (group) o.push_back("-DRS_JIT_GROUP=1");
  if (group && resident) o.push_back("-DRS_JIT_GROUP_RESIDENT=1");
  if (group && queued && !counted) o.push_back("-DRS_JIT_GROUP_QUEUED=1");
  if (group && counted) o.push_back("-DRS_JIT_GROUP_COUNTED=1");
  if (group && flows) o.push_back("-DRS_JIT_GROUP_FLOWS=1");
  if (group && resident && run) o.push_back("-DRS_JIT_GROUP_RUN=1");
  if (sched == 11) o.push_back("-fno-slp-vectorize");
  if (tuned) {
    o.push_back("-mllvm");
    o.push_back("-amdgpu-atomic-optimizer-strategy=None");
    std::string vforce;
    if (variant)
      if (const char* q = strstr(variant, "ss=")) { vforce = q + 3; vforce = vforce.substr(0, vforce.find(' ')); }
    const char* const force = !vforce.empty() ? vforce.c_str() : getenv("RS_JIT_SCHED_STRATEGY");
    if (force) {
      if (strcmp(force, "default") != 0) { o.push_back("-mllvm"); o.push_back(std::string("-amdgpu-sched-strategy=") + force); }
    } else if (!qmode && !direct && (sched == 9 || (sched == 8 && (R > 32 || win > 0)))) {
      o.push_back("-mllvm");
      o.push_back("-amdgpu-sched-strategy=iterative-ilp");
    }
  }
  for (int pass = 0; pass < 2; ++pass) {
    const char* extra = pass == 0 ? getenv("RS_JIT_EXTRA") : variant;
    if (!extra) continue;
    std::string e(extra);
    size_t pos = 0;
    while (pos < e.size()) {
      size_t sp = e.find(' ', pos);
      if (sp == std::string::npos) sp = e.size();
      if (sp > pos && e.compare(pos, 3, "ss=") != 0) o.push_back(e.substr(pos, sp - pos));
      pos = sp + 1;
    }
  }
  return o;
}

static std::mutex g_hiprtc_mu;
static std::vector<char> rs_jit_compile_opts(const std::vector<std::string>& o, std::string& log) {
  std::lock_guard<std::mutex> one_at_a_time(g_hiprtc_mu);
  std::vector<char> code;
  hiprtcProgram prog;
  const char* hdr_src[kRsJitNumHeaders];
  const char* hdr_name[kRsJitNumHeaders];
  for (int i = 0; i < kRsJitNumHeaders; ++i) { hdr_src[i] = kRsJitHeaders[i].text; hdr_name[i] = kRsJitHeaders[i].name; }
  if (hiprtcCreateProgram(&prog, kRsJitKernelsHip, "rs_kernels.hip", kRsJitNumHeaders, hdr_src, hdr_name) != HIPRTC_SUCCESS) {
    log = "hiprtcCreateProgram failed";
    return code;
  }
  std::vector<const char*> opts;
  for (auto& s : o) opts.push_back(s.c_str());
  hiprtcResult r = hiprtcCompileProgram(prog, (int)opts.size(), opts.data());
  if (r != HIPRTC_SUCCESS) {
    size_t ls = 0;
// ... 154 lines not shown
    if (fread(&klen, 8, 1, f) != 1 || klen != key_text.size()) break;
    k.resize(klen);
    if (fread(&k[0], 1, klen, f) != klen || k != key_text) break;
    if (fread(&clen, 8, 1, f) != 1 || fread(&sum, 8, 1, f) != 1 || clen == 0 || clen > (64ull << 20)) break;
    code.resize(clen);
    if (fread(code.data(), 1, clen, f) != clen || fread(mark, 1, 8, f) != 8 || fgetc(f) != EOF) break;
    ok = fnv1a(code.data(), clen) == sum;
    if (verified) *verified = ok && memcmp(mark, kMarkVerified, 8) == 0;
  } while (false);
  fclose(f);
  if (!ok) { code.clear(); g_cache_rejected++; }
  return ok;
}

void cache_store(const std::string& file, const std::string& key_text, const std::vector<char>& code) {
  const size_t slash = file.rfind('/');
  if (slash == std::string::npos || !make_dirs(file.substr(0, slash))) return;
  static std::atomic<unsigned> seq{0};
  const std::string tmp = file + "." + std::to_string((long long)getpid()) + "." + std::to_string(seq++) + ".tmp";
  const int fd = open(tmp.c_str(), O_WRONLY | O_CREAT | O_EXCL, 0600);
  FILE* f = fd >= 0 ? fdopen(fd, "wb") : nullptr;
  if (!f) { if (fd >= 0) close(fd); return; }
  const unsigned long long klen = key_text.size(), clen = code.size(), sum = fnv1a(code.data(), code.size());
  const bool ok = fwrite(kCacheMagic, 1, 6, f) == 6 && fwrite(&klen, 8, 1, f) == 1 && fwrite(key_text.data(), 1, klen, f) == klen &&
                  fwrite(&clen, 8, 1, f) == 1 && fwrite(&sum, 8, 1, f) == 1 && fwrite(code.data(), 1, clen, f) == clen &&
                  fwrite(kMarkUnchecked, 1, 8, f) == 8;
  if (fclose(f) != 0 || !ok || rename(tmp.c_str(), file.c_str()) != 0) { (void)unlink(tmp.c_str()); return; }
  g_cache_stores++;
}
}

static std::vector<char> rs_jit_code(const std::vector<std::string>& opts, std::string& log, std::string* file_out = nullptr,
                                     std::string* key_out = nullptr, bool* from_cache = nullptr, bool* verified = nullptr) {
  if (from_cache) *from_cache = false;
  if (verified) *verified = false;
  if (!cache_enabled()) return rs_jit_compile_opts(opts, log);
  const std::string key_text = cache_key_text(opts), file = cache_file_of(key_text);
  if (file_out) *file_out = file;
  if (key_out) *key_out = key_text;
  std::vector<char> code;
  if (!file.empty() && cache_load(file, key_text, code, verified)) {
    g_cache_hits++;
    if (from_cache) *from_cache = true;
    return code;
  }
  g_cache_misses++;
  code = rs_jit_compile_opts(opts, log);
  if (!code.empty() && !file.empty()) cache_store(file, key_text, code);
  return code;
}

static bool rs_jit_queued_sched(int sched) { return sched == 7 || sched == 8 || sched == 9 || sched == 101 || sched == 103; }
static const char* rs_jit_group_flags_error(int flags, int sched) {
  if ((flags & 256) != 0 && ((flags & 8) == 0 || (flags & 16) == 0))
    return "flag value 256 (the run form) is valid only together with 8 (a group's build) and 16 (the resident form)";
  if ((flags & 256) != 0 && (flags & (32 | 64 | 128)) != 0)
    return "flag value 256 (the run form) excludes 32 (the queued form), 64 (the counted form) and 128 (the flows form)";
  if ((flags & 256) != 0 && (sched == 7 || sched == 11)) return "flag value 256 (the run form) does not exist for schedulers 7 and 11";
  if ((flags & 128) != 0 && (flags & 8) == 0) return "flag value 128 (the flows form) is valid only together with 8 (a group's build)";
  if ((flags & 128) != 0 && (flags & (16 | 32 | 64)) != 0)
    return "flag value 128 (the flows form) excludes 16 (the resident form), 32 (the queued form) and 64 (the counted form)";
  if ((flags & 128) != 0 && sched != 1) return "flag value 128 (the flows form) exists for scheduler 1 only";
  if ((flags & 64) != 0 && ((flags & 8) == 0 || (flags & 32) == 0))
    return "flag value 64 (the counted form) is valid only together with 8 (a group's build) and 32 (the queued form)";
  if ((flags & 16) != 0 && (flags & 8) == 0) return "flag value 16 (the resident form) is valid only together with 8 (a group's build)";
  if ((flags & 32) != 0 && (flags & 8) == 0) return "flag value 32 (the queued form) is valid only together with 8 (a group's build)";
  if ((flags & 32) != 0 && (flags & 16) != 0) return "flag values 16 (the resident form) and 32 (the queued form) exclude each other";
  if ((flags & 32) != 0 && !rs_jit_queued_sched(sched)) return "flag value 32 (the queued form) exists for schedulers 7, 8, 9, 101 and 103 only";
  return nullptr;
}

extern "C" const char* rs_jit_compiler_identity(void) { return compiler_identity().c_str(); }

extern "C" void rs_jit_cache_stats(long long out[4]) {
  out[0] = g_cache_hits; out[1] = g_cache_misses; out[2] = g_cache_stores; out[3] = g_cache_rejected;
}

extern "C" int rs_jit_cache_file(int S, int U, int R, int G, int NT, int sched, int flags, char* out, size_t outlen) {
  if (rs_jit_group_flags_error(flags, sched)) {
    if (out && outlen) out[0] = 0;
    return 0;
  }
  const std::vector<std::string> o = rs_jit_options(S, U, R, G, NT, sched, 0, equal_slices_window(S, U), true, (flags & 1) != 0 || (flags & 8) != 0, (flags & 2) != 0, (flags & 4) != 0, nullptr, (flags & 8) != 0, (flags & 16) != 0, (flags & 32) != 0, (flags & 64) != 0, (flags & 128) != 0, (flags & 256) != 0);
  const std::string file = cache_file_of(cache_key_text(o));
  if (out && outlen) snprintf(out, outlen, "%s", file.c_str());
  return (int)file.size();
}

extern "C" int rs_jit_cache_warm(int S, int U, int R, int G, int NT, int sched, int flags, char* err, size_t errlen) {
  std::string log;
  if (const char* why = rs_jit_group_flags_error(flags, sched)) {
    if (err && errlen) snprintf(err, errlen, "%s", why);
    return -1;
  }
  const std::vector<char> code = rs_jit_code(rs_jit_options(S, U, R, G, NT, sched, 0, equal_slices_window(S, U), true, (flags & 1) != 0 || (flags & 8) != 0, (flags & 2) != 0, (flags & 4) != 0, nullptr, (flags & 8) != 0, (flags & 16) != 0, (flags & 32) != 0, (flags & 64) != 0, (flags & 128) != 0, (flags & 256) != 0), log);
  if (code.empty()) {
    if (err && errlen) snprintf(err, errlen, "%.*s", (int)errlen - 1, log.c_str());
    return -1;
  }
  return (int)code.size();
}

extern "C" int rs_jit_selfcheck(int S, int U, int R, int G, int NT, int sched, char* err, size_t errlen) {
  std::string log;
  std::vector<char> code = rs_jit_compile(S, U, R, G, NT, sched, log, 0, equal_slices_window(S, U));
  if (code.empty()) {
    if (err && errlen) snprintf(err, errlen, "%.*s", (int)errlen - 1, log.c_str());
    return -1;
  }
  return (int)code.size();
}

extern "C" int rs_jit_selfcheck_untuned(int S, int U, int R, int G, int NT, int sched, char* err, size_t errlen) {
  std::string log;
  std::vector<char> code = rs_jit_compile(S, U, R, G, NT, sched, log, 0, equal_slices_window(S, U), false);
  if (code.empty()) {
    if (err && errlen) snprintf(err, errlen, "%.*s", (int)errlen - 1, log.c_str());
    return -1;
  }
  return (int)code.size();
}

extern "C" int rs_jit_selfcheck_dropin(int S, int U, int R, int G, int NT, int sched, char* err, size_t errlen) {
  std::string log;
  const int qmode = (sched == 1 || sched == 7) ? 1 : 0;
  std::vector<char> code = rs_jit_compile(S, U, R, G, NT, sched, log, qmode, 0, true, true);
  if (code.empty()) {
    if (err && errlen) snprintf(err, errlen, "%.*s", (int)errlen - 1, log.c_str());
    return -1;
  }
  return (int)code.size();
}

static int selfcheck_group_pair(int S, int U, int R, int G, int NT, int sched, bool resident, char* err, size_t errlen, bool queued = false,
                                bool counted = false, bool flows = false, bool run = false) {
  const int qmode = (sched == 1 || sched == 7) ? 1 : 0;
  int largest = 0;
  for (int lean = 0; lean < 2; ++lean) {
    std::string log;
    std::vector<char> code = rs_jit_compile(S, U, R, G, NT, sched, log, qmode, 0, true, true, false, lean != 0, true, resident, queued, counted, flows, run);
    if (code.empty()) {
      if (err && errlen) snprintf(err, errlen, "%s build: %.*s", lean ? "lean" : "general", errlen > 16 ? (int)errlen - 16 : 0, log.c_str());
      return -1;
    }
    largest = (int)code.size() > largest ? (int)code.size() : largest;
  }
  return largest;
}
// ... 8 lines not shown

extern "C" int rs_jit_selfcheck_group_queued(int S, int U, int R, int G, int NT, int sched, char* err, size_t errlen) {
  if (!rs_jit_queued_sched(sched)) {
    if (err && errlen) snprintf(err, errlen, "scheduler %d has no queued form (rs_group_queued_kernel exists for 7, 8, 9, 101 and 103)", sched);
    return -1;
  }
  return selfcheck_group_pair(S, U, R, G, NT, sched, false, err, errlen, true);
}

extern "C" int rs_jit_selfcheck_group_counted(int S, int U, int R, int G, int NT, int sched, char* err, size_t errlen) {
  if (!rs_jit_queued_sched(sched)) {
    if (err && errlen) snprintf(err, errlen, "scheduler %d has no counted form (rs_group_counted_kernel exists for 7, 8, 9, 101 and 103)", sched);
    return -1;
  }
  return selfcheck_group_pair(S, U, R, G, NT, sched, false, err, errlen, true, true);
}

extern "C" int rs_jit_selfcheck_group_flows(int S, int U, int R, int G, int NT, int sched, char* err, size_t errlen) {
  if (sched != 1) {
    if (err && errlen) snprintf(err, errlen, "scheduler %d has no flows form (rs_group_flows_kernel exists for scheduler 1)", sched);
    return -1;
  }
  return selfcheck_group_pair(S, U, R, G, NT, sched, false, err, errlen, false, false, true);
}

extern "C" int rs_jit_selfcheck_group_run(int S, int U, int R, int G, int NT, int sched, char* err, size_t errlen) {
  if (sched == 7 || sched == 11) {
    if (err && errlen) snprintf(err, errlen, "scheduler %d has no run form (rs_group_run_kernel exists for 1, 8, 9, 10, 101 and 103)", sched);
    return -1;
  }
  return selfcheck_group_pair(S, U, R, G, NT, sched, true, err, errlen, false, false, false, true);
}

extern "C" int rs_jit_selfcheck_queue(int S, int U, int R, int G, int NT, int sched, char* err, size_t errlen) {
  std::string log;
  std::vector<char> code = rs_jit_compile(S, U, R, G, NT, sched, log, 2);
  if (code.empty()) {
    if (err && errlen) snprintf(err, errlen, "%.*s", (int)errlen - 1, log.c_str());
    return -1;
  }
  return (int)code.size();
}

extern "C" RsJitKernel* rs_jit_get(int device, int S, int U, int R, int G, int NT, int sched, int qmode, int win, char* err, size_t errlen,
                                   int flags, const char* variant) {
  const bool group = (flags & 8) != 0;
  const bool resident = (flags & 16) != 0;
  const bool queued = (flags & 32) != 0;
  const bool counted = (flags & 64) != 0;
  const bool flows = (flags & 128) != 0;
  const bool run = (flags & 256) != 0;
  if (const char* why = rs_jit_group_flags_error(flags, sched)) {
    if (err && errlen) snprintf(err, errlen, "shape-specialised kernel unavailable (flags: %s)", why);
    return nullptr;
  }
  const int direct = (flags & 1) | (group ? 1 : 0);
  const bool streamed = (flags & 2) != 0;
  const bool lean = (flags & 4) != 0;
  char shape[128];
  snprintf(shape, sizeof shape, "d%d S%d U%d R%d G%d NT%d s%d q%d w%d x%d ", device, S, U, R, G, NT, sched, qmode, win, flags);
  const std::string key = std::string(shape) + (getenv("RS_JIT_EXTRA") ? getenv("RS_JIT_EXTRA") : "") +
                          (getenv("RS_JIT_SCHED_STRATEGY") ? std::string(" ss=") + getenv("RS_JIT_SCHED_STRATEGY") : std::string()) +
                          (variant ? std::string(" v[") + variant + "]" : std::string());
  std::lock_guard<std::mutex> lock(g_mu);
  auto failmsg = [&](const char* what, const char* detail) {
    if (err && errlen) snprintf(err, errlen, "shape-specialised kernel unavailable (%s: %.300s)", what, detail ? detail : "");
    return (RsJitKernel*)nullptr;
  };
  auto it = g_cache.find(key);
  if (it != g_cache.end()) {
    if (it->second->rejected) return failmsg("self-check", "this build disagreed with the built-in kernels earlier in this process and was dropped");
    return it->second;
  }
  std::string log, file, key_text;
  bool untuned = false, from_cache = false, verified = false;
  std::vector<char> code = rs_jit_code(rs_jit_options(S, U, R, G, NT, sched, qmode, win, true, direct != 0, streamed, lean, variant, group, resident, queued, counted, flows, run), log, &file, &key_text,
                                       &from_cache, &verified);
  if (code.empty() && !getenv("RS_JIT_NO_RETRY")) {
    std::string log2;
    code = rs_jit_code(rs_jit_options(S, U, R, G, NT, sched, qmode, win, false, direct != 0, streamed, lean, variant, group, resident, queued, counted, flows, run), log2, &file, &key_text, &from_cache,
                       &verified);
    untuned = !code.empty();
  }
  if (code.empty()) return failmsg("hiprtc", log.c_str());
  RsJitKernel* k = new RsJitKernel();
  k->threads = NT;
  k->untuned = untuned;
  k->from_cache = from_cache;
  k->verified = verified;
  k->cache_file = file;
  k->key_text = key_text;
  k->what = key;
  const RsCarve cv = rs_carve(S, U, R, sched, NT, qmode, win);
  k->lds_bytes = cv.lds_bytes;
  k->q_lds = cv.q_lds;
  hipError_t e = hipModuleLoadData(&k->mod, code.data());
  if (e != hipSuccess) { delete k; return failmsg("hipModuleLoadData", hipGetErrorString(e)); }
  e = hipModuleGetFunction(&k->fn, k->mod, !group ? "rs_cell_kernel_jit" : run ? "rs_group_run_kernel_jit" : resident ? "rs_group_resident_kernel_jit" : counted ? "rs_group_counted_kernel_jit" : flows ? "rs_group_flows_kernel_jit" : queued ? "rs_group_queued_kernel_jit" : "rs_group_kernel_jit");
  if (e != hipSuccess) { (void)hipModuleUnload(k->mod); delete k; return failmsg("hipModuleGetFunction", hipGetErrorString(e)); }
  g_cache[key] = k;
  return k;
}

extern "C" int rs_jit_is_verified(const RsJitKernel* k) { return k && k->verified ? 1 : 0; }
extern "C" int rs_jit_was_loaded(const RsJitKernel* k) { return k && k->from_cache ? 1 : 0; }

extern "C" void rs_jit_mark_verified(RsJitKernel* k) {
  if (!k || k->rejected) return;
  std::lock_guard<std::mutex> lock(g_mu);
  if (k->verified) return;
  k->verified = true;
  if (k->cache_file.empty() || !cache_enabled()) return;
  std::vector<char> code;
  bool marked = false;
  const long long rejected_before = g_cache_rejected;
  if (!cache_load(k->cache_file, k->key_text, code, &marked)) { g_cache_rejected = rejected_before; return; }
  if (marked) return;
  const int fd = open(k->cache_file.c_str(), O_WRONLY);
  if (fd < 0) return;
  const off_t end = lseek(fd, 0, SEEK_END);
  if (end >= 8 && pwrite(fd, kMarkVerified, 8, end - 8) != 8) {  }
  close(fd);
}

extern "C" void rs_jit_reject(RsJitKernel* k) {
  if (!k) return;
  std::lock_guard<std::mutex> lock(g_mu);
  k->rejected = true;
  k->verified = false;
  if (!k->cache_file.empty()) (void)unlink(k->cache_file.c_str());
}

extern "C" int rs_jit_is_untuned(const RsJitKernel* k) { return k && k->untuned ? 1 : 0; }
// ... 12 lines not shown
```

### radiosaber_amd/csrc/rs_kernels.hip

```cpp
#ifndef __HIPCC_RTC__
#include <hip/hip_runtime.h>
#include <stdint.h>
#endif

#include "rs_device.h"
#include "rs_sort_emul.h"
#include "rs_wave.h"
#include "rs_sort_device.h"
#include "rs_interslice.h"

namespace {

#ifndef RS_P3_BLOCK_TOP
#define RS_P3_BLOCK_TOP 0
#endif
template <int N> struct RsInt { static constexpr int v = N; };

__device__ __forceinline__ double rs_div_1000(double x) {
  const double q = x * 0.001;
  const double r = __builtin_fma(-q, 1000.0, x);
  return __builtin_fma(r, 0.001, q);
}
#ifndef RS_PRIO_WINDOW_LOG2
#define RS_PRIO_WINDOW_LOG2 15
// ... 4 lines not shown
    else __builtin_amdgcn_s_setprio(x);                                      \
  } while (0)
#define RS_SPEC_NAP 2
#define RS_SERIAL_PRIO 3
#ifndef RS_SPEC_PRIO
#define RS_SPEC_PRIO 0
#endif
#ifndef RS_P3_BLOCK
#define RS_P3_BLOCK 32
#endif

#ifdef RS_STAMPS
#define RS_STAMP(i)                                                \
  do {                                                             \
    if (tid == 0) {                                                \
      unsigned long long now_ = __builtin_readcyclecounter();      \
      stamp_acc[i] += now_ - stamp_prev;                           \
      stamp_prev = now_;                                           \
    }                                                              \
  } while (0)
#else
#define RS_STAMP(i) do { } while (0)
#endif
#ifndef RS_STAMPS_W1_TID
#define RS_STAMPS_W1_TID 64
#endif
#if defined(RS_STAMPS) && defined(RS_STAMPS_W1)
#define RS_STAMP1(i)                                               \
  do {                                                             \
    if (tid == RS_STAMPS_W1_TID) {                                 \
      unsigned long long now_ = __builtin_readcyclecounter();      \
      sort_sub[i] += now_ - stamp1_prev;                           \
      stamp1_prev = now_;                                          \
    }                                                              \
  } while (0)
#else
#define RS_STAMP1(i) do { } while (0)
#endif

#ifndef RS_JIT_S
#define RS_JIT_S 1
#define RS_JIT_U 1
#define RS_JIT_R 1
#define RS_JIT_G 1
#define RS_JIT_NT 64
#define RS_JIT_SCHED 8
#endif
#ifndef RS_JIT_WIN
#define RS_JIT_WIN 0
#endif
#ifndef RS_JIT_CARVEQ
#define RS_JIT_CARVEQ 0
#endif

template <int SCHED, int EPT, bool FIXED, bool DIRECT, bool QUEUE = false, bool GROUP = false>
__device__ __forceinline__ void rs_cell_body(const RsLaunch& p, unsigned char* lds) {
  static_assert(!GROUP || (DIRECT && !QUEUE && SCHED != 11), "group calls: the one-TTI form (built in, or a group's run-time build), scheduler 11 excepted");
  static_assert(!QUEUE || (!DIRECT && (SCHED == 8 || SCHED == 9 || SCHED == 101 || SCHED == 103 || SCHED == 1 || SCHED == 7)),
                "finite queues: batches of schedulers 1, 7, 8, 9, 101, 103");
  constexpr bool kQSerial = QUEUE && (SCHED == 1 || SCHED == 7);
  const int cell = GROUP ? 0 : blockIdx.x;
#ifdef RS_STAMPS
  const unsigned long long stamp_entry = __builtin_readcyclecounter();
#endif
  constexpr bool kDirect = DIRECT;
  const bool per_prb = DIRECT ? p.prb_cqi != nullptr : (p.epochs_prb != nullptr || p.trace_prb != nullptr);
  const int queue_mode_in = DIRECT ? p.queue_mode : (QUEUE ? 1 : 0);
  constexpr RsCarve kCvQ = rs_carve(RS_JIT_S, RS_JIT_U, RS_JIT_R, RS_JIT_SCHED, RS_JIT_NT, RS_JIT_CARVEQ, RS_JIT_WIN);
  const bool q_lds = QUEUE && (FIXED ? kCvQ.q_lds != 0 : p.q_lds != 0);
  const int qU = FIXED ? RS_JIT_U : p.U;
  unsigned char* const qs = lds + (FIXED ? kCvQ.off_qstate : p.off_qstate);
  double* const qs_avg = (double*)qs;
  double* const qs_next = qs_avg + 2 * qU;
  double* const qs_headt = qs_next + 2 * qU;
  double* const qs_hol = qs_headt + 2 * qU;
  int32_t* const qs_i = (int32_t*)(qs_hol + qU);
  long long* const qs_a0 = (long long*)(qs_i + 14 * qU);
  int32_t* const qs_narr = (int32_t*)(qs_a0 + 2 * qU);
  int32_t* const qs_hnf = qs_narr + 2 * qU;
  int32_t* const qs_hla = qs_hnf + 2 * qU;
  uint8_t* const qs_kind = (uint8_t*)(qs_hla + 2 * qU);
  uint8_t* const qs_flags = qs_kind + 2 * qU;
  uint8_t* const qs_slice = qs_flags + qU;
  const uint8_t* const prio_in = QUEUE ? (q_lds ? qs_flags : p.q_flags + (size_t)blockIdx.x * qU) : (DIRECT ? p.prio : nullptr);
  const double* const hol_in = QUEUE ? (q_lds ? qs_hol : p.q_hol + (size_t)blockIdx.x * qU) : (DIRECT ? p.hol : nullptr);
  const int tid = threadIdx.x;
  const int nt = FIXED ? RS_JIT_NT : (int)blockDim.x;
  const int lane = lane_id(), wave = wave_id(), nwaves = nt >> 6;
  const int S = FIXED ? RS_JIT_S : p.S, U = (FIXED && !DIRECT) ? RS_JIT_U : p.U, R = FIXED ? RS_JIT_R : p.R, G = FIXED ? RS_JIT_G : p.G;
  constexpr RsCarve kCv = rs_carve(RS_JIT_S, RS_JIT_U, RS_JIT_R, RS_JIT_SCHED, RS_JIT_NT, RS_JIT_CARVEQ, RS_JIT_WIN);
  struct Offs { int avgk, rcp, tab, slice, tx, misc, tbs, elems, sorted, items, sortx, cqi, queue, Upad, n_seg, n_items; };
  const Offs o = FIXED ? Offs{kCv.off_avgk, kCv.off_rcp, kCv.off_tab, kCv.off_slice, kCv.off_tx, kCv.off_misc, kCv.off_tbs,
                              kCv.off_elems, kCv.off_sorted, kCv.off_items, kCv.off_sortx, kCv.off_cqi, kCv.off_queue,
                              DIRECT ? p.Upad : kCv.Upad, DIRECT ? p.n_seg : kCv.n_seg, DIRECT ? p.n_items : kCv.n_items}
                       : Offs{p.off_avgk, p.off_rcp, p.off_tab, p.off_slice, p.off_tx, p.off_misc, p.off_tbs, p.off_elems,
                              p.off_sorted, p.off_items, p.off_sortx, p.off_cqi, p.off_queue, p.Upad, p.n_seg, p.n_items};
  constexpr bool kTransport = (SCHED == 8 || SCHED == 9 || SCHED == 101 || SCHED == 103 || SCHED == 10);
  const int quota_wave = nwaves - 1;
#ifndef RS_VEC_MAX_R
#define RS_VEC_MAX_R 32
#endif
  constexpr int kVecMaxR = RS_VEC_MAX_R;
  constexpr bool kVecScan = SCHED == 9 && (!FIXED || RS_JIT_R <= kVecMaxR);
  const bool vec_scan = kVecScan && R <= kVecMaxR;
#if defined(RS_NO_HOLD)
  constexpr bool kHoldSched = false;
#elif defined(RS_HOLD_ALWAYS)
  constexpr bool kHoldSched = FIXED && RS_JIT_NT <= 512 && !DIRECT && !QUEUE && (SCHED == 8 || SCHED == 9 || SCHED == 101 || SCHED == 103);
#else
  constexpr bool kHoldSched = FIXED && RS_JIT_R <= 32 && RS_JIT_NT <= 512 && !DIRECT && !QUEUE &&
                              (SCHED == 8 || SCHED == 101 || SCHED == 103 || (SCHED == 9 && RS_JIT_WIN > 0 && RS_JIT_WIN <= 64));
#endif
#ifdef RS_NO_SPEC
  constexpr bool kSpecSched = false;
#else
  constexpr bool kSpecSched = !kHoldSched && !DIRECT && !QUEUE && (SCHED == 8 || SCHED == 9 || SCHED == 101 || SCHED == 103) &&
                              (!FIXED || RS_JIT_U <= 32 * RS_JIT_S) && !(FIXED && kVecScan);
#endif
  const bool spec_enabled = kSpecSched && nwaves >= 2 && U <= 32 * S && !vec_scan;
#ifdef RS_NO_EARLY17
  constexpr bool kEarly17 = false;
#else
  constexpr bool kEarly17 = FIXED && !DIRECT && !QUEUE && (SCHED == 7 || (SCHED == 1 && RS_JIT_U > RS_JIT_NT));
#endif
#if defined(RS_NO_PF1_LANES)
  constexpr bool kPf1 = false;
#elif defined(RS_PF1_ALWAYS)
  constexpr bool kPf1 = FIXED && !DIRECT && !QUEUE && SCHED == 1 && RS_JIT_U <= 2048;
#else
  constexpr bool kPf1 = FIXED && !DIRECT && !QUEUE && SCHED == 1 && RS_JIT_U > 512 && RS_JIT_U <= 2048;
#endif
  constexpr bool kQuad7 = kEarly17 && SCHED == 7 && kCv.nvs_seg == 0 && RS_JIT_WIN > 0 && RS_JIT_WIN <= 64;

  double* s_avg = (double*)lds;
  double* s_avgk = (double*)(lds + o.avgk);
  float* s_rcp32 = (float*)(lds + o.rcp);
  int32_t* s_tx = (int32_t*)(lds + o.tx);
  double* s_num = (double*)(lds + o.tab);
  double* s_e = s_num + 16;
  double* s_x = s_e + 16;
  float* s_num32 = (float*)(s_x + 16);
  double* s_w = (double*)(lds + o.slice);
  double* s_sstate = s_w + 64;
  uint16_t* s_best_user = (uint16_t*)(lds + o.items);
  double* s_best_metric = (double*)(lds + o.elems);
  uint32_t* s_elems = (uint32_t*)(lds + o.elems);
  uint32_t* s_sorted = (uint32_t*)(lds + o.sorted);
  Misc* m = (Misc*)(lds + o.misc);
  int32_t* s_tbs = (int32_t*)(lds + o.tbs);
  uint8_t* s_cqi = lds + o.cqi;
  const int Upad = o.Upad;

  const RsTables* tab = p.tab;
  RsCellScalars* scal = p.scal + cell;
  if (!DIRECT && tid == 0) {
    scal->clk_begin = __builtin_readcyclecounter();
    scal->real_begin = __builtin_amdgcn_s_memrealtime();
  }

  constexpr bool kCumRegs = FIXED && !DIRECT && !QUEUE;
  constexpr int kKU = kCumRegs ? (RS_JIT_U + RS_JIT_NT - 1) / RS_JIT_NT : 1;
  int cum_b[kKU], cum_r[kKU];
#pragma unroll
  for (int k = 0; k < kKU; ++k) { cum_b[k] = 0; cum_r[k] = 0; }
  constexpr int kPU = (FIXED && DIRECT) ? (RS_JIT_U + RS_JIT_NT - 1) / RS_JIT_NT : 1;
  constexpr int kPGsrc = (FIXED && DIRECT) ? ((RS_JIT_U * RS_JIT_R + 15) / 16 + RS_JIT_NT - 1) / RS_JIT_NT : 1;
  constexpr int kPGimg = (FIXED && DIRECT) ? ((rs_upad_of(RS_JIT_U) * RS_JIT_R + 15) / 16 + RS_JIT_NT - 1) / RS_JIT_NT : 1;
  constexpr int kPG = kPGsrc > kPGimg ? kPGsrc : kPGimg;
  constexpr bool kPrefetch = FIXED && DIRECT && SCHED == 9 && kPG <= 2;
  const bool grid_from_image = DIRECT && p.image_mode == 2;
  double pre_avg[kPU];
  int pre_sl[kPU];
  uint4 pre_grid[kPG];
  if constexpr (kPrefetch) {
    const uint4* src = grid_from_image ? (const uint4*)p.grid_image : (const uint4*)p.epochs;
    const int n16 = grid_from_image ? (R * (int)p.Upad + 15) >> 4 : (int)(p.grid_stride >> 4);
#pragma unroll
    for (int k = 0; k < kPU; ++k) {
      const int u = tid + k * nt;
      pre_avg[k] = u < U ? p.avg[u] : 0.0;
      pre_sl[k] = u < U ? (int)p.user_slice[u] : 0;
    }
#pragma unroll
    for (int j = 0; j < kPG; ++j) {
      const int i = tid + j * nt;
      pre_grid[j] = i < n16 ? src[i] : make_uint4(0u, 0u, 0u, 0u);
    }
  }
#pragma unroll
  for (int ku = 0; ku < (kCumRegs ? kKU : 1); ++ku) {
    if (!kCumRegs) break;
    const int u = tid + ku * nt;
    if (u < U) {
      s_avg[u] = p.avg[(size_t)cell * U + u];
      int v = p.tx_bytes[(size_t)cell * U + u];
      if (v & RS_TX_COUNTED) {
        cum_b[ku] -= v & RS_TX_BYTES_MASK;
        cum_r[ku] -= (v >> RS_TX_NPRB_SHIFT) & RS_TX_NPRB_MASK;
        v &= ~RS_TX_COUNTED;
      }
      s_tx[u] = v;
    }
  }
  for (int u = tid; u < U && !kCumRegs; u += nt) {
    if (!kPrefetch) s_avg[u] = p.avg[(size_t)cell * U + u];
    s_tx[u] = kDirect ? 0 : p.tx_bytes[(size_t)cell * U + u];
    if (kDirect) {
      if (p.log_tbs) p.log_tbs[u] = 0;
      if (p.log_uinfo) p.log_uinfo[u] = 0;
    }
  }
  int16_t* const s_uoff = (int16_t*)(s_rcp32 + Upad + 16 * S);
  if constexpr (kPrefetch) {
#pragma unroll
    for (int k = 0; k < kPU; ++k) {
      const int u = tid + k * nt;
      if (u < U) { s_avg[u] = pre_avg[k]; s_uoff[u] = (int16_t)pre_sl[k]; }
    }
  }
  for (int i = tid; i < (R + 1) * 16; i += nt) s_tbs[i] = p.tbs_eff[i];
  if (!grid_from_image)
    for (int i = tid; i < (R * Upad) >> 2; i += nt) ((uint32_t*)s_cqi)[i] = 0;
  for (int i = tid; i < Upad + 16 * S; i += nt) s_rcp32[i] = 0.0f;
  if (tid < 16) {
    s_num[tid] = (SCHED == 1 || SCHED == 11) ? tab->pfnum[tid] : tab->kbps[tid];
    s_e[tid] = tab->eesm_e[tid];
    s_x[tid] = tab->eesm_x[tid];
    s_num32[tid] = (float)((SCHED == 1 || SCHED == 11) ? tab->pfnum[tid] : tab->kbps[tid]);
    m->mcs_of_cqi[tid] = tab->mcs_of_cqi[tid];
    m->tbs1_of_cqi[tid] = tab->tbs1_syn[tid];
    m->ones16[tid] = 1.0f;
    m->eff16[tid] = tab->eff[tid];
  }
  if (tid < 2) { m->spec[tid].ctr_p1 = 0; m->spec[tid].ctr_p3 = 0; m->spec[tid].greedy_done = 0; m->spec[tid].n_fix = 0; }
  if (tid == 0) m->grid_free = 0;
  if ((SCHED == 9 || SCHED == 10) && tid < 3) m->heap_sorts[tid] = 0;
  if (tid < S) {
    m->eps_psi[tid] = (uint8_t)((p.eps[tid] ? 1 : 0) | (p.psi[tid] ? 2 : 0) | ((p.alpha && p.alpha[tid]) ? 4 : 0) | ((p.beta && p.beta[tid]) ? 8 : 0));
    s_w[tid] = p.weight[tid];
    s_sstate[tid] = p.slice_state[(size_t)cell * S + tid];
  }
  if (SCHED == 1) {
    if (tid <= o.n_seg) m->seg_begin[tid] = min(tid * RS_PF_SEG, U);
  } else {
    if (tid <= S) m->seg_begin[tid] = U;
  }
  __syncthreads();
  if (SCHED != 1) {
    for (int u = tid; u < U; u += nt) {
      int s = kPrefetch ? (int)s_uoff[u] : (int)p.user_slice[u];
      int sp = u == 0 ? -1 : (kPrefetch ? (int)s_uoff[u - 1] : (int)p.user_slice[u - 1]);
      for (int q = sp + 1; q <= s; q++) m->seg_begin[q] = u;
    }
  }
  if (SCHED != 1) {
    __syncthreads();
    if (wave == 0) {
      const int ub = lane < S ? m->seg_begin[lane] : 0, ue = lane < S ? m->seg_begin[lane + 1] : 0;
      const int wl = ue > ub ? ((ue + 7) & ~7) - (ub & ~7) : 0;
      const int wb = wave_scan_incl(wl) - wl;
      if (lane < S) m->rcp_off[lane] = wb - (ub & ~7);
    }
    __syncthreads();
    if constexpr (kPrefetch) {
#pragma unroll
      for (int k = 0; k < kPU; ++k) {
        const int u = tid + k * nt;
        if (u < U) s_uoff[u] = (int16_t)(m->rcp_off[pre_sl[k]] | ((m->eps_psi[pre_sl[k]] & 2) ? 1 : 0));
      }
    } else {
      for (int u = tid; u < U; u += nt) s_uoff[u] = (int16_t)(m->rcp_off[p.user_slice[u]] | (p.psi[p.user_slice[u]] ? 1 : 0));
    }
  }
// ... 281 lines not shown
  constexpr int kGrpSched = SCHED, kGrpEpt = EPT;
  constexpr bool kGrpFixed = false, kGrpLean = false, kGrpRes = false, kGrpQue = true, kGrpCnt = false, kGrpFlow = false, kGrpRun = false;
#include "rs_phase_group.inc"
}

template <int SCHED, int EPT>
__global__ void __launch_bounds__(512, 4) rs_group_counted_kernel(RsLaunch p) {
  extern __shared__ __align__(16) unsigned char lds[];
  constexpr int kGrpSched = SCHED, kGrpEpt = EPT;
  constexpr bool kGrpFixed = false, kGrpLean = false, kGrpRes = false, kGrpQue = true, kGrpCnt = true, kGrpFlow = false, kGrpRun = false;
#include "rs_phase_group.inc"
}

template <int SCHED, int EPT>
__global__ void __launch_bounds__(512, 4) rs_group_flows_kernel(RsLaunch p) {
  extern __shared__ __align__(16) unsigned char lds[];
  constexpr int kGrpSched = SCHED, kGrpEpt = EPT;
  constexpr bool kGrpFixed = false, kGrpLean = false, kGrpRes = false, kGrpQue = false, kGrpCnt = false, kGrpFlow = true, kGrpRun = false;
#include "rs_phase_group.inc"
}

template <int SCHED, int EPT>
__global__ void __launch_bounds__(512, 4) rs_group_run_kernel(RsLaunch p) {
  extern __shared__ __align__(16) unsigned char lds[];
  constexpr int kGrpSched = SCHED, kGrpEpt = EPT;
  constexpr bool kGrpFixed = false, kGrpLean = false, kGrpRes = true, kGrpQue = false, kGrpCnt = false, kGrpFlow = false, kGrpRun = true;
#include "rs_phase_group.inc"
}
#else
#ifndef RS_JIT_DIRECT
#define RS_JIT_DIRECT 0
#endif
#ifndef RS_JIT_WPE
#define RS_JIT_WPE 4
#endif
#ifndef RS_JIT_GROUP
#define RS_JIT_GROUP 0
#endif
#ifndef RS_JIT_GROUP_RESIDENT
#define RS_JIT_GROUP_RESIDENT 0
#endif
#ifndef RS_JIT_GROUP_QUEUED
#define RS_JIT_GROUP_QUEUED 0
#endif
#ifndef RS_JIT_GROUP_COUNTED
#define RS_JIT_GROUP_COUNTED 0
#endif
#ifndef RS_JIT_GROUP_FLOWS
#define RS_JIT_GROUP_FLOWS 0
#endif
#ifndef RS_JIT_GROUP_RUN
#define RS_JIT_GROUP_RUN 0
#endif
#if RS_JIT_GROUP
#if RS_JIT_GROUP_RESIDENT && RS_JIT_GROUP_QUEUED
#error "RS_JIT_GROUP_RESIDENT and RS_JIT_GROUP_QUEUED exclude each other"
#endif
#if RS_JIT_GROUP_RESIDENT && RS_JIT_GROUP_COUNTED
#error "RS_JIT_GROUP_RESIDENT and RS_JIT_GROUP_COUNTED exclude each other"
#endif
#if RS_JIT_GROUP_FLOWS && (RS_JIT_GROUP_RESIDENT || RS_JIT_GROUP_QUEUED || RS_JIT_GROUP_COUNTED)
#error "RS_JIT_GROUP_FLOWS is never combined with RS_JIT_GROUP_RESIDENT, RS_JIT_GROUP_QUEUED or RS_JIT_GROUP_COUNTED"
#endif
#if RS_JIT_GROUP_FLOWS && RS_JIT_SCHED != 1
#error "RS_JIT_GROUP_FLOWS: the flows form is scheduler 1's"
#endif
#if RS_JIT_GROUP_RUN && !RS_JIT_GROUP_RESIDENT
#error "RS_JIT_GROUP_RUN needs RS_JIT_GROUP_RESIDENT: the run form is the resident form's"
#endif
#if RS_JIT_GROUP_RUN && (RS_JIT_GROUP_QUEUED || RS_JIT_GROUP_COUNTED || RS_JIT_GROUP_FLOWS)
#error "RS_JIT_GROUP_RUN is never combined with RS_JIT_GROUP_QUEUED, RS_JIT_GROUP_COUNTED or RS_JIT_GROUP_FLOWS"
#endif
#if RS_JIT_GROUP_RUN && RS_JIT_SCHED == 7
#error "RS_JIT_GROUP_RUN: scheduler 7 has no run form (the host picks the served slice per TTI)"
#endif
#if RS_JIT_GROUP_RUN
#define RS_GROUP_JIT_ENTRY rs_group_run_kernel_jit
#elif RS_JIT_GROUP_RESIDENT
#define RS_GROUP_JIT_ENTRY rs_group_resident_kernel_jit
#elif RS_JIT_GROUP_COUNTED
#define RS_GROUP_JIT_ENTRY rs_group_counted_kernel_jit
#elif RS_JIT_GROUP_FLOWS
#define RS_GROUP_JIT_ENTRY rs_group_flows_kernel_jit
#elif RS_JIT_GROUP_QUEUED
#define RS_GROUP_JIT_ENTRY rs_group_queued_kernel_jit
#else
#define RS_GROUP_JIT_ENTRY rs_group_kernel_jit
#endif
extern "C" __global__ void __launch_bounds__(RS_JIT_NT, RS_JIT_WPE) RS_GROUP_JIT_ENTRY(RsLaunch p) {
#if defined(RS_JIT_LEAN) && RS_JIT_LEAN
  p.cqi_mode = RS_CQI_EPOCHS;
  p.prb_cqi = nullptr; p.queue_mode = 0; p.alpha = nullptr; p.beta = nullptr; p.hol = nullptr; p.prio = nullptr;
#if !RS_JIT_GROUP_FLOWS
  p.gate = nullptr;
#endif
  p.exact_scan = 0; p.gen_exp = 0; p.gen_num = nullptr; p.log_upper = nullptr; p.synthetic = 0;
  p.trace = nullptr; p.trace_prb = nullptr; p.epochs_prb = nullptr; p.log_keys = nullptr;
  constexpr bool kGrpLean = true;
#else
  constexpr bool kGrpLean = false;
#endif
  constexpr RsCarve kCv = rs_carve(RS_JIT_S, RS_JIT_U, RS_JIT_R, RS_JIT_SCHED, RS_JIT_NT, RS_JIT_CARVEQ, RS_JIT_WIN);
  __shared__ __align__(16) unsigned char lds[kCv.lds_bytes];
  constexpr int kGrpSched = RS_JIT_SCHED, kGrpEpt = (RS_JIT_SCHED != 9 && RS_JIT_SCHED != 10) ? 0 : (kCv.ept <= 4 ? kCv.ept : 0);
  constexpr bool kGrpFixed = true, kGrpRes = RS_JIT_GROUP_RESIDENT != 0, kGrpQue = RS_JIT_GROUP_QUEUED != 0 || RS_JIT_GROUP_COUNTED != 0,
                 kGrpCnt = RS_JIT_GROUP_COUNTED != 0, kGrpFlow = RS_JIT_GROUP_FLOWS != 0, kGrpRun = RS_JIT_GROUP_RUN != 0;
#include "rs_phase_group.inc"
}
#undef RS_GROUP_JIT_ENTRY
#else
extern "C" __global__ void __launch_bounds__(RS_JIT_NT, RS_JIT_WPE) rs_cell_kernel_jit(RsLaunch p) {
#if defined(RS_JIT_LEAN) && RS_JIT_LEAN && !RS_JIT_DIRECT
  p.cqi_mode = RS_CQI_EPOCHS;
  p.trace = nullptr; p.trace_prb = nullptr; p.epochs_prb = nullptr; p.user_trace = nullptr;
  p.log_map = nullptr; p.log_quota = nullptr; p.log_target = nullptr; p.log_tbs = nullptr; p.log_uinfo = nullptr; p.log_keys = nullptr;
  p.log_bbytes = nullptr; p.log_bhol = nullptr;
  p.phy_draws = 0; p.synthetic = 0;
#elif defined(RS_JIT_LEAN) && RS_JIT_LEAN
  p.cqi_mode = RS_CQI_EPOCHS;
  p.prb_cqi = nullptr; p.queue_mode = 0; p.alpha = nullptr; p.beta = nullptr; p.hol = nullptr; p.prio = nullptr;
  p.gate = nullptr; p.exact_scan = 0; p.gen_exp = 0; p.gen_num = nullptr; p.log_upper = nullptr; p.synthetic = 0;
  p.trace = nullptr; p.trace_prb = nullptr; p.epochs_prb = nullptr; p.log_keys = nullptr;
#endif
  constexpr RsCarve kCv = rs_carve(RS_JIT_S, RS_JIT_U, RS_JIT_R, RS_JIT_SCHED, RS_JIT_NT, RS_JIT_CARVEQ, RS_JIT_WIN);
  __shared__ __align__(16) unsigned char lds[kCv.lds_bytes];
  constexpr int kEpt = (RS_JIT_SCHED != 9 && RS_JIT_SCHED != 10) ? 0 : (kCv.ept <= 4 ? kCv.ept : 0);
  rs_cell_body<RS_JIT_SCHED, kEpt, true, RS_JIT_DIRECT != 0, (RS_JIT_CARVEQ >= 2)>(p, lds);
}
#endif
#endif

__device__ __forceinline__ uint64_t splitmix64(uint64_t z) {
  z += 0x9E3779B97F4A7C15ull;
  z = (z ^ (z >> 30)) * 0xBF58476D1CE4E5B9ull;
  z = (z ^ (z >> 27)) * 0x94D049BB133111EBull;
  return z ^ (z >> 31);
}

struct RsCdf {
  uint32_t c[16];
};

__global__ void rs_synth_cqi_kernel(uint8_t* epochs, int64_t grid_stride, int n_cells, int n_epochs, int U,
                                    int R, int Upad, uint64_t seed, int64_t first_cell, RsCdf cdf) {
  const int64_t grids = (int64_t)n_cells * n_epochs;
  const int64_t per_grid16 = grid_stride >> 4;
  const int64_t total = grids * per_grid16;
  for (int64_t w = (int64_t)blockIdx.x * blockDim.x + threadIdx.x; w < total; w += (int64_t)gridDim.x * blockDim.x) {
    int64_t g = w / per_grid16;
    int64_t o = (w - g * per_grid16) << 4;
    uint8_t out[16];
    int r = (int)(o / Upad), u = (int)(o - (int64_t)r * Upad);
#pragma unroll
    for (int k = 0; k < 16; ++k) {
      uint8_t v = 0;
      if (r < R && u < U) {
        const int64_t idx = (int64_t)u * R + r;
        const uint64_t gcell = (uint64_t)(first_cell + g / n_epochs), ep = (uint64_t)(g % n_epochs);
        uint64_t h = splitmix64(seed ^ splitmix64(splitmix64(gcell * 0x100000001B3ull + ep) + (uint64_t)idx));
        uint32_t x = (uint32_t)(h >> 32);
        int q = 0;
#pragma unroll
        for (int j = 0; j < 14; ++j) q += x > cdf.c[j] ? 1 : 0;
        v = (uint8_t)(q + 1);
      }
      out[k] = v;
      if (++u == Upad) { u = 0; ++r; }
    }
    *(uint4*)(epochs + g * grid_stride + o) = *(const uint4*)out;
  }
}

__global__ void __launch_bounds__(256) rs_copy_probe_kernel(const uint4* __restrict__ src, uint4* __restrict__ dst, size_t n16) {
  const size_t stride = (size_t)gridDim.x * blockDim.x;
  for (size_t i = (size_t)blockIdx.x * blockDim.x + threadIdx.x; i < n16; i += stride) dst[i] = src[i];
}

// ... 301 lines not shown
```

### radiosaber_amd/csrc/rs_phase_p3.inc

```
    const int nvs_seg = FIXED ? kCv.nvs_seg : p.nvs_seg;
    int nvs_lo = 0, nvs_hi = 0, nvs_first = 0;
    const bool nvs_split = SCHED == 7 && nvs_seg != 0;
    if (nvs_split) {
      nvs_lo = kDirect ? 0 : m->seg_begin[seg_lo];
      nvs_hi = kDirect ? U : m->seg_begin[seg_lo + 1];
      nvs_first = nvs_lo & ~7;
      nvs_runs = idiv_small(nvs_hi - nvs_first + nvs_seg - 1, nvs_seg);
    }
    const int n_items = nvs_split ? R * nvs_runs : o.n_items;
    auto scan_item = [&](int it, uint16_t* bu_out, uint32_t* rec_out, auto blk_tag) -> bool {
      bool held = false;
      float top1 = 0.0f, top2 = 0.0f;
      {
        int sg = it / R, r = it - sg * R;
        int seg = SCHED == 7 ? seg_lo : sg;
        int ub = m->seg_begin[seg], ue = m->seg_begin[seg + 1];
        if (SCHED == 7 && kDirect) { ub = 0; ue = U; }
        if (nvs_split) {
          ub = nvs_first + sg * nvs_seg;
          ue = ub + nvs_seg;
          ub = ub < nvs_lo ? nvs_lo : ub;
          ue = ue > nvs_hi ? nvs_hi : ue;
        }
        double best = SCHED == 1 ? 0.0 : (SCHED == 7 ? -1.7976931348623157e308 : -1.0);
        int bu = -1;
        float run_a = 0.0f;
        bool exact = false;
        int sl_eps = 1, sl_psi = 1;
        int sl_custom = 0;
        int sl_id = 0;
        if (SCHED != 1) {
          int sl = SCHED == 7 ? (kDirect ? (int)p.user_slice[0] : seg) : seg;
          sl_id = sl;
          sl_eps = m->eps_psi[sl] & 1;
          sl_psi = (m->eps_psi[sl] >> 1) & 1;
          if (queue_mode_in && (m->eps_psi[sl] & 4)) sl_custom = (SCHED == 7 || (m->eps_psi[sl] & 8) != 0) ? 2 : 1;
        }
        const uint8_t* rowp = s_cqi + r * Upad;
        const float kTol = 0x1.ffffcp-1f;
        constexpr int kP3Block = decltype(blk_tag)::v != 0 ? decltype(blk_tag)::v
                                 : (SCHED == 7 && FIXED && kCv.nvs_seg != 0) ? kCv.nvs_seg
                                 : ((kSpecSched && RS_P3_BLOCK > 16) ? 16 : RS_P3_BLOCK);
        const bool one_num = SCHED != 1 && !sl_eps;
        const float* numtab = one_num ? m->ones16 : s_num32;
        const float* rcw = s_rcp32 + (SCHED == 1 ? 0 : m->rcp_off[(SCHED == 7 && kDirect) ? (int)p.user_slice[0] : seg]);
        auto exact_metric = [&](int u, int c) -> double {
          if (SCHED == 1) {
            return s_num[c] / s_avg[u];
          }
          const double num_c = s_num[c], den_u = s_avgk[u];
          double num = sl_eps ? num_c : 1.0, den = sl_psi ? den_u : 1.0;
          if constexpr (DIRECT) {
            if (p.gen_exp) { num = p.gen_num[sl_id * 16 + c]; den = den_u; }
          }
          if (QUEUE && (prio_in[u] & 2) == 0) return -2.0;
          if (sl_custom && prio_in && (prio_in[u] & 1) == 0) return 0.0;
          if (sl_custom == 2) return hol_in[u] * num / den;
          return num / den;
        };
        if constexpr (DIRECT) {
          if (p.exact_scan) {
            for (int u = ub; u < ue; ++u) {
// ... 57 lines not shown
                while (cand) {
                  const int j = __ffs((int)cand) - 1;
                  cand &= cand - 1;
                  const int u = blk + j;
                  const double metric = exact_metric(u, rowp[u]);
                  if (metric > best) { best = metric; bu = u; }
                }
                exact = true;
                run_a = *(const float*)((const char*)numtab + ((uint32_t)rowp[bu] << 2)) * rcw[bu];
              }
            }
          } else {
            const float thr = best_a > 0.0f ? best_a * kTol : __builtin_inff();
            uint32_t cand = 0;
#pragma unroll
            for (int k = 0; k < kP3Block; ++k) cand |= av[k] >= thr ? (1u << k) : 0u;
            if (!cand) {
              if (QUEUE) {
#pragma unroll
                for (int k = 0; k < kP3Block; ++k) cand |= (blk + k >= ub && blk + k < ue) ? (1u << k) : 0u;
              } else {
                cand = 1u << ((ub > blk ? ub : blk) - blk);
              }
            }
            while (cand) {
              const int j = __ffs((int)cand) - 1;
              cand &= cand - 1;
              const int u = blk + j;
              const double metric = exact_metric(u, rowp[u]);
              if (metric > best) { best = metric; bu = u; }
            }
            exact = true;
          }
        }
        const int bkey = bu >= 0 ? rowp[bu] : 0;
        if ((SCHED == 1 || nvs_split) && !exact && bu >= 0) best = exact_metric(bu, bkey);
        bu_out[it] = (uint16_t)bu;
        if constexpr (kHoldSched) {
          if (bu >= 0) {
            if (!sl_psi) {
              held = true;
            } else {
              const float la = *(const float*)((const char*)numtab + ((uint32_t)bkey << 2)) * rcw[bu];
              const double aw = s_avg[bu];
              const float mu = 0x1p-18f + 2.0f / (1.0f + (float)aw);
              held = aw >= 64.0 && la >= top1 && top2 * (1.0f + mu) * 1.000001f <= la;
            }
          }
        }
        if (SCHED == 10) {
          rec_out[sg * R + r] = ((uint32_t)bkey << 16) | ((uint32_t)r << 8) | (uint32_t)sg;
        } else if (kTransport) {
          rec_out[r * S + sg] = ((uint32_t)bkey << 16) | ((uint32_t)r << 8) | (uint32_t)sg;
        } else if (SCHED == 1 || nvs_split) {
          s_best_metric[it] = best;
        }
      }
      return held;
    };
    if constexpr (kQSerial && SCHED == 7) {
      const int ub = m->seg_begin[seg_lo], ue = m->seg_begin[seg_lo + 1];
      for (int u = ub + tid; u < ue; u += nt) {
        int need = 0;
        if (prio_in[u] & 2) {
          double sum = 0;
          if (per_prb) {
            for (int r = 0; r < R; ++r) {
              const uint8_t* pr = prb_ptr(u, r);
              for (int k = 0; k < G; ++k) sum += s_e[pr[k]];
            }
          } else {
            for (int r = 0; r < R; ++r) {
              const double ev = s_e[s_cqi[r * Upad + u]];
              for (int k = 0; k < G; ++k) sum += ev;
            }
          }
          const double x = sum / (double)(R * G);
          int wide = 15;
          if (!(x == 0)) {
            wide = 1;
#pragma unroll
            for (int k = 1; k <= 13; ++k) wide += (x <= xthr_k[k - 1]) ? 1 : 0;
          }
          const int first = q_data0[u] > 0 ? q_data0[u] : q_data1[u];
          need = (first * 8) / tab->tbs1_of_cqi[wide];
        }
        q_need[u] = need;
      }
      if (ue - ub <= 64 && (ue - ub) * 128 <= o.items - o.elems) {
        const int sl_eps7 = m->eps_psi[seg_lo] & 1, sl_psi7 = (m->eps_psi[seg_lo] >> 1) & 1;
        const bool custom7 = (m->eps_psi[seg_lo] & 4) != 0;
        double* const qt = (double*)s_elems;
        for (int i = tid; i < (ue - ub) * 16; i += nt) {
          const int u = ub + (i >> 4), cq = i & 15;
          const double num = sl_eps7 ? s_num[cq] : 1.0, den = sl_psi7 ? s_avgk[u] : 1.0;
          qt[i] = !custom7 ? num / den : ((prio_in[u] & 1) == 0 ? 0.0 : hol_in[u] * num / den);
        }
      }
    }
    struct QuadWinner { bool writer; int user, bits; float la, g1, g2; };
    constexpr bool kQuadScan = kHoldSched || kQuad7;
    constexpr int kMaxGrp = (FIXED && RS_JIT_WIN > 0 && RS_JIT_WIN <= 32) ? 1 : 2;
    auto quad_scan = [&](const bool on, const int sg, const int r) -> QuadWinner {
      const float kTolH = 0x1.ffffcp-1f;
      const int q4 = lane & 3;
      const int ngrp = kMaxGrp == 1 ? 1 : (hold_win <= 32 ? 1 : 2);
// ... 72 lines not shown
              const int mhi = quad_max_i(bhi);
              const int mlo = quad_max_i(bhi == mhi ? blo : (int)0x80000000);
              const unsigned long long eq = __ballot(on && cnt > 1 && bhi == mhi && blo == mlo);
              const unsigned quad = (unsigned)(eq >> (lane & ~3)) & 0xfu;
              if (on && cnt > 1 && (quad & ((1u << q4) - 1u)) == 0u && ((quad >> q4) & 1u)) {
                writer = true;
                ul = bu_l;
                la = numtab[rowp[bu_l]] * rcw[bu_l];
              }
            }
      return QuadWinner{writer, ul, bits, la, g1, g2};
    };
    (void)kQuadScan;
    bool hold_full = true;
    if constexpr (kHoldSched) {
      bool full = !hold_ok || tti == 0 || grid_loaded || hold_age >= RS_HOLD_MAX_AGE;
      int hold_listed = 0;
#if defined(RS_STAMPS) && defined(RS_STAMPS_HOLD)
      unsigned long long hs_prev = __builtin_readcyclecounter();
#define RS_HSTAMP(i) do { if (tid == 0) { unsigned long long n_ = __builtin_readcyclecounter(); sort_sub[i] += n_ - hs_prev; hs_prev = n_; } } while (0)
#else
#define RS_HSTAMP(i) do { } while (0)
#endif
      if (!full) {
        const int grp = lane >> 2;
        uint16_t* const wl = hold_wl;
        for (int k0 = 0; k0 * nwaves < n_items; k0 += 64) {
          const int n_list = (pre_listed >= 0 && k0 == 0) ? pre_listed : hold_pack(k0, wave);
          hold_listed += n_list;
          RS_HSTAMP(0);
          constexpr int kHoldPrio = SCHED == 8 ? 1 : 0;
          if (kHoldPrio) RS_SETPRIO(kHoldPrio);
          for (int base = 0; base < n_list; base += 16) {
            const bool on = base + grp < n_list;
            const int it = on ? (int)wl[base + grp] : 0;
            const int sg = FIXED ? it / RS_JIT_R : idiv_small(it, R), r = it - sg * R;
            const QuadWinner w = quad_scan(on, sg, r);
            const bool writer = w.writer;
            const int ul = w.user, bits = w.bits;
            const float la = w.la, g1 = w.g1, g2 = w.g2;
            const uint8_t* rowp = s_cqi + r * Upad;
            if (writer) {
              const int key = rowp[ul];
              bool held = false;
              if (!(bits & 2)) {
                held = true;
              } else {
                const double aw = s_avg[ul];
                const float mu = 0x1p-18f + 2.0f / (1.0f + (float)aw);
                held = aw >= 64.0 && la >= g1 && g2 * (1.0f + mu) * 1.000001f <= la;
              }
              cur_bu[it] = (uint16_t)ul;
              if (SCHED != 9) cur_rec[r * S + sg] = ((uint32_t)key << 16) | ((uint32_t)r << 8) | (uint32_t)sg;
              const int kk = FIXED ? it / (RS_JIT_NT / 64) : idiv_small(it, nwaves);
              unsigned long long* const word = &hold_bits[(kk >> 6) * nwaves + wave];
              if (held) atomicOr(word, 1ull << (kk & 63));
              else atomicAnd(word, ~(1ull << (kk & 63)));
            }
          }
          __builtin_amdgcn_fence(__ATOMIC_ACQ_REL, "wavefront");
          __builtin_amdgcn_wave_barrier();
          if (kHoldPrio) RS_SETPRIO(0);
          RS_HSTAMP(1);
        }
        hold_age += 1;
      }
      if (full) {
        for (int k0 = 0; k0 * nwaves < n_items; k0 += 64) {
          const int j = (k0 + lane) * nwaves + wave;
          bool held = false;
          if (j < n_items) held = scan_item(j, cur_bu, cur_rec, RsInt<RS_P3_BLOCK_TOP>{});
          const unsigned long long hm = __ballot(held);
          if (hold_ok && lane == 0) hold_bits[(k0 >> 6) * nwaves + wave] = hm;
        }
        hold_age = 0;
      }
      hold_full = full;
      pre_listed = -1;
#ifdef RS_STAMPS
      if (tid == 0) sort_sub[6] += (unsigned long long)hold_listed + ((unsigned long long)(full ? 1 : 0) << 32);
#endif
    } else
    if constexpr (kPf1) {
      constexpr int kUL = (((RS_JIT_U + 63) / 64) + 7) & ~7;
      static_assert(kUL <= 32, "per-flow PF lanes: five position bits");
      const float kTol16 = 0x1.fffep-1f;
      const int u_first = kUL * lane;
      float rcl[kUL];
#pragma unroll
      for (int q = 0; q < kUL / 4; ++q) {
        float4 rv = make_float4(0.f, 0.f, 0.f, 0.f);
        if (u_first + 4 * q < U) rv = *(const float4*)(s_rcp32 + u_first + 4 * q);
        rcl[4 * q] = rv.x; rcl[4 * q + 1] = rv.y; rcl[4 * q + 2] = rv.z; rcl[4 * q + 3] = rv.w;
      }
      auto settle_exactly = [&](int r, int thr) -> int {
        const uint8_t* rowp = s_cqi + r * Upad;
        double best = 0.0;
        int bu = -1;
#pragma unroll 1
        for (int k = 0; k < kUL; ++k) {
          const int u = u_first + k;
          if (u < U) {
            const int c = rowp[u];
            const int w = (__float_as_int(s_num32[c] * s_rcp32[u]) & ~31) | (31 - k);
            if (w >= thr) {
              const double metric = s_num[c] / s_avg[u];
// ... 95 lines not shown
```

### radiosaber_amd/csrc/rs_phase_p4.inc

```
    if (SCHED == 9) {
      const int N = R * S;
      {
        uint16_t* sx = (uint16_t*)(lds + o.sortx);
        uint16_t* pa = (uint16_t*)s_sorted;
        RS_SETPRIO(1);
        if constexpr (kHoldSched) {
          if (!hold_full) {
            for (int x = tid; x < N; x += nt) {
              const int r = FIXED ? x / RS_JIT_S : idiv_small(x, S), sg = x - r * S;
              const int bu = cur_bu[sg * R + r];
              const uint32_t key = bu == 0xFFFF ? 0u : (uint32_t)s_cqi[r * Upad + bu];
              s_elems[x] = (key << 16) | ((uint32_t)r << 8) | (uint32_t)sg;
            }
            if (EPT == 0) __syncthreads();
          }
        }
        if constexpr (EPT > 0) introsort_levels_reg<EPT, FIXED ? RS_JIT_NT : 0>(s_elems, N, s_sorted, (int32_t*)sx, m, sort_sub, 0,
                                                                           rs_sort_ranks_bytes(N) ? (uint16_t*)(lds + o.sortx + rs_sort_cuts_bytes(N)) : m->hist);
        else introsort_loop_levels(s_elems, N, pa, pa + N, sx, sx + N, sx + 2 * N, sx + 3 * N, m);
      }
      RS_STAMP(3);
      RS_SETPRIO(2);
      if constexpr (EPT > 0) counting_sort_desc_owned<EPT, FIXED ? RS_JIT_NT : 0>(s_elems, s_sorted, N, m);
      else counting_sort_desc(s_elems, s_sorted, N, m);
      RS_SETPRIO(0);
      RS_STAMP(4);
    }
    if constexpr (SCHED == 10) {
      static_assert(EPT > 0, "UpperBound uses the register form of the sort (R*S <= 4 * threads)");
      const int N = R * S;
      RS_SETPRIO(1);
      introsort_levels_reg<EPT, FIXED ? RS_JIT_NT : 0>(s_elems, N, s_sorted, (int32_t*)(lds + o.sortx), m, sort_sub, R,
                                                       rs_sort_ranks_bytes(N) ? (uint16_t*)(lds + o.sortx + rs_sort_cuts_bytes(N)) : m->hist);
      RS_SETPRIO(0);
      int32_t* low_owner = (int32_t*)m->hist;
      if (R > 32) {
        uint32_t* const cnt = (uint32_t*)m->maskA + wave * 16;
        const unsigned long long gt_lane = lane == 63 ? 0ull : (~0ull << (lane + 1));
        for (int sl = wave; sl < S; sl += nwaves) {
          const int f = sl * R;
          const bool valid = lane < R;
          const uint32_t e = valid ? s_elems[f + lane] : 0u;
          const int k = (int)(e >> 16);
          if (lane < 16) cnt[lane] = 0u;
          uint32_t dl = 0u, dh = 0u;
#pragma unroll
          for (int b = 0; b < 4; ++b) {
            const uint32_t mine = (uint32_t)(((int)(e << (15 - b))) >> 31);
            const unsigned long long plane = __ballot(mine != 0u);
            dl |= (uint32_t)plane ^ mine;
            dh |= (uint32_t)(plane >> 32) ^ mine;
          }
          const unsigned long long vm = __ballot(valid);
          const uint32_t sl_ = (uint32_t)vm & ~dl, sh_ = (uint32_t)(vm >> 32) & ~dh;
          const int rank_eq = (int)__builtin_amdgcn_mbcnt_hi(sh_, __builtin_amdgcn_mbcnt_lo(sl_, 0u));
          if (valid && ((sl_ & (uint32_t)gt_lane) | (sh_ & (uint32_t)(gt_lane >> 32))) == 0u) cnt[k] = (uint32_t)(rank_eq + 1);
          int inc = lane < 16 ? (int)cnt[lane] : 0;
          {
            int v_ = inc;
            const int identity = 0;
// ... 110 lines not shown
```

### radiosaber_amd/csrc/rs_phase_p5.inc

```
      constexpr bool kFlows = kQSerial && SCHED == 1;
#if defined(RS_STAMPS) && defined(RS_STAMPS_P5)
      unsigned long long p5_prev = __builtin_readcyclecounter();
#define RS_P5STAMP(i) do { if (tid == 0) { unsigned long long n_ = __builtin_readcyclecounter(); sort_sub[i] += n_ - p5_prev; p5_prev = n_; } } while (0)
#else
#define RS_P5STAMP(i) do { } while (0)
#endif
      const uint8_t* const col = s_cqi + (owner < 0 ? 0 : (kFlows ? owner >> 1 : owner));
      double ev_mine = 0.0;
      if (kTransport && !per_prb) {
        const double ev = s_e[col[(lane < R ? lane : 0) * Upad]];
        ev_mine = (lane < R && owner >= 0) ? ev : 0.0;
      }
      unsigned long long same = 0ull;
      {
        const bool has = lane < R && owner >= 0;
        const int key = has ? owner + 1 : 0;
        if constexpr (!(FIXED && kVecScan)) {
          m->maskA[lane] = 0ull;
          m->maskB[lane] = 0ull;
          __builtin_amdgcn_fence(__ATOMIC_ACQ_REL, "wavefront");
          __builtin_amdgcn_wave_barrier();
        }
        if (has) {
          atomicOr(&m->maskA[key & 63], 1ull << lane);
// ... 66 lines not shown
                for (int k = 0; k < G; ++k) sum += ev[i];
                nprb += G;
              }
            if (pair2) {
#pragma unroll
              for (int i = 2; i < 4; ++i)
                if (more[i]) {
                  for (int k = 0; k < G; ++k) sum += ev[i];
                  nprb += G;
                }
            }
          }
          mm = 0ull;
        }
        while (mm) {
          const int r2 = __ffsll((long long)mm) - 1;
          mm &= mm - 1;
          if (per_prb) {
            const uint8_t* pr = prb_ptr(kFlows ? owner >> 1 : owner, r2);
            for (int k = 0; k < G; ++k) sum += s_e[pr[k]];
          } else {
            const double ev = s_e[col[r2 * Upad]];
            for (int k = 0; k < G; ++k) sum += ev;
          }
          nprb += G;
        }
        RS_P5STAMP(2);
        int syn_bits = 0;
        if (p.synthetic && (SCHED == 7 || kTransport)) {
          int t1 = 0;
          if (lane < R && owner >= 0) {
            if (per_prb) {
              const uint8_t* pr = prb_ptr(owner, lane);
              for (int k = 0; k < G; ++k) t1 += m->tbs1_of_cqi[pr[k]];
            } else {
              t1 = G * m->tbs1_of_cqi[col[lane * Upad]];
            }
          }
          unsigned long long ms = leader ? same : 0ull;
          while (__ballot(ms != 0ull) != 0ull) {
            const bool more = ms != 0ull;
            const int r2 = more ? __ffsll((long long)ms) - 1 : 0;
            ms &= ms - 1;
            const int v = __shfl(t1, r2, 64);
            if (more) syn_bits += v;
          }
        }
        RS_P5STAMP(3);
        if (kGridAhead && grid_next) {
          __builtin_amdgcn_fence(__ATOMIC_RELEASE, "workgroup");
          if (lane == 0) __hip_atomic_store(&m->grid_free, tti + 1, __ATOMIC_RELAXED, __HIP_MEMORY_SCOPE_WORKGROUP);
        }
        if (leader) {
          const double x = sum / (double)nprb;
          if (x == 0) {
            fcqi = 15;
          } else {
            fcqi = 1;
#pragma unroll
            for (int k = 1; k <= 13; ++k) fcqi += (x <= xthr_k[k - 1]) ? 1 : 0;
          }
          RS_P5STAMP(4);
          mcs = m->mcs_of_cqi[fcqi];
          tbs = (p.synthetic && (SCHED == 7 || kTransport)) ? syn_bits : s_tbs[(nprb / G) * 16 + fcqi];
          int bytes = tbs / 8;
          if (bytes > 100000000) bytes = 100000000;
#if defined(RS_FAULT_INJECT_JIT) || (defined(RS_FAULT_INJECT_P3B8) && RS_P3_BLOCK == 8) || (defined(RS_FAULT_INJECT_LEAN) && defined(RS_JIT_LEAN) && RS_JIT_LEAN)
          if (FIXED && bytes > 0) bytes += 1;
#endif
          if (bytes > 0) {
            if (kFlows) {
              if (owner & 1) q_grant1[owner >> 1] = bytes | (nprb << RS_TX_NPRB_SHIFT);
              else s_tx[owner >> 1] = bytes | (nprb << RS_TX_NPRB_SHIFT);
            } else if (kCumRegs || QUEUE) {
              atomicAdd(&s_tx[owner], bytes | (nprb << RS_TX_NPRB_SHIFT));
            } else {
              if (!(kSpecSched && spec_next)) s_tx[owner] += bytes;
              if (!DIRECT) {
                atomicAdd((unsigned long long*)&p.cum_bytes[(size_t)cell * U + owner], (unsigned long long)bytes);
                atomicAdd((unsigned long long*)&p.cum_rbs[(size_t)cell * U + owner], (unsigned long long)nprb);
              }
            }
          }
          if ((kSpecSched && spec_next) || (kHoldSched && ewma_next) || early17) tbs_bytes_next = bytes;
        }
      }
      RS_P5STAMP(5);
      if ((kHoldSched && ewma_next) || early17) {
        while (rs_lds_load(&fl_cur->ctr_p1) < nwaves - 1) __builtin_amdgcn_s_sleep(1);
        __builtin_amdgcn_fence(__ATOMIC_ACQUIRE, "workgroup");
        if (leader) {
          const double t_next = t + 0.001;
          const double dt_next = t_next - t;
          double a = SCHED == 1 ? s_avgk[owner] : s_avg[owner];
          const double rate = (double)(tbs_bytes_next * 8) / dt_next;
          const double beta = 0.02;
          a = a + (beta * rate);
          if (a < 1) a = 1;
          s_avg[owner] = a;
          if (SCHED == 1) s_rcp32[owner] = __builtin_amdgcn_rcpf((float)a);
          else pf_terms(owner, a);
        }
      }
      if (kSpecSched && spec_next) {
        RS_STAMP(7);
        while (rs_lds_load(&fl_cur->ctr_p3) < nwaves - 1) __builtin_amdgcn_s_sleep(1);
        __builtin_amdgcn_fence(__ATOMIC_ACQUIRE, "workgroup");
        RS_STAMP(6);
        if (leader) {
          const double t_next = t + 0.001;
          const double dt_next = t_next - t;
          double a = s_avg[owner];
          const double rate = (double)(tbs_bytes_next * 8) / dt_next;
// ... 28 lines not shown
```

Before: 43.59 million.

## Add roomy LDS carve with precomputed link-adaptation thresholds and pristine sort records

Adds an optional larger LDS layout for batch kernels. It holds a per-allocation-size table of exact sum thresholds, so the CQI mapping compares the raw sum against precomputed bounds and skips the double division. It also holds a copy of the first-pass sort records, so phase 4 copies them instead of rebuilding keys from cur_bu. The layout is on by default when the doubled LDS still fits and the cell count is small, which trades extra LDS use (and possibly occupancy) for less per-TTI arithmetic.

```diff
diff --git a/include/radiosaber_hip.h b/include/radiosaber_hip.h
--- a/include/radiosaber_hip.h
+++ b/include/radiosaber_hip.h
@@ -61,6 +61,7 @@
 int rs_link_tables(double eff[16], double kbps[16], double eesm_e[16], double eesm_x[16]);
 int rs_link_tables_pinned(double eff[16], double kbps[16], double eesm_e[16], double eesm_x[16]);
 int rs_link_tables_compare(char* msg, size_t msglen);
+int rs_link_y_table(int link_tables, int n_rbgs, int rbg_size, double* y);
 
 int rs_get_rbg_size(int nb_rbs);
 int rs_dl_prbs_for_bandwidth(double bw_mhz);
diff --git a/radiosaber_amd/__init__.py b/radiosaber_amd/__init__.py
--- a/radiosaber_amd/__init__.py
+++ b/radiosaber_amd/__init__.py
@@ -6,7 +6,7 @@
     RS_SCHED_MAXCELL, RS_SCHED_NVS, RS_SCHED_PF, RS_SCHED_NVS_NONGREEDY, RS_SCHED_SEQUENTIAL, RS_SCHED_UPPERBOUND, RS_SCHED_VOGEL, RS_SCHED_SUBOPT,
     BEARER_BACKLOG, BEARER_NONE, BEARER_QUEUE, FULL_PACKET, TRACE_CQI_HISTOGRAM, frames_to_bursts, internet_flow_arrivals,
     BatchScheduler, GroupScheduler, RadioSaberError, SliceConfig, TtiResult, TtiScheduler, device_count, device_source_hash, dl_prbs_for_bandwidth, get_rbg_size, hbm_copy_probe, jit_selfcheck, lds_bytes_per_cell,
-    jit_cache_file, jit_cache_stats, jit_cache_warm, jit_compiler_identity, lib, link_tables_compare,
+    jit_cache_file, jit_cache_stats, jit_cache_warm, jit_compiler_identity, lib, link_tables_compare, link_y_table,
     RS_LINK_DEFAULT, RS_LINK_HOST_LIBM, RS_LINK_PINNED_GLIBC_2_35,
     link_tables, load_trace_dir, read_trace_mapping, read_ue_trace,
 )
@@ -16,4 +16,4 @@
            "link_tables", "jit_selfcheck", "device_source_hash", "TRACE_CQI_HISTOGRAM", "read_trace_mapping", "read_ue_trace",
            "load_trace_dir", "hbm_copy_probe", "lds_bytes_per_cell", "get_rbg_size", "dl_prbs_for_bandwidth", "internet_flow_arrivals", "frames_to_bursts",
            "BEARER_NONE", "BEARER_BACKLOG", "BEARER_QUEUE", "FULL_PACKET", "jit_cache_file", "jit_cache_stats", "jit_cache_warm",
-           "jit_compiler_identity", "link_tables_compare", "RS_LINK_DEFAULT", "RS_LINK_HOST_LIBM", "RS_LINK_PINNED_GLIBC_2_35"]
+           "jit_compiler_identity", "link_tables_compare", "link_y_table", "RS_LINK_DEFAULT", "RS_LINK_HOST_LIBM", "RS_LINK_PINNED_GLIBC_2_35"]
diff --git a/radiosaber_amd/api.py b/radiosaber_amd/api.py
--- a/radiosaber_amd/api.py
+++ b/radiosaber_amd/api.py
@@ -91,7 +91,7 @@
     "rs_batch_debug_heap_sorts", "rs_ctx_debug_heap_sorts",
     "rs_jit_cache_stats", "rs_jit_cache_file", "rs_jit_cache_warm", "rs_batch_autotune_report", "rs_batch_debug_clocks",
     "rs_batch_checkpoint_bytes", "rs_batch_checkpoint_save", "rs_batch_checkpoint_load",
-    "rs_link_tables_pinned", "rs_link_tables_compare", "rs_ctx_jit_status", "rs_jit_compiler_identity",
+    "rs_link_tables_pinned", "rs_link_tables_compare", "rs_link_y_table", "rs_ctx_jit_status", "rs_jit_compiler_identity",
     "rs_batch_flow_record", "rs_batch_run_logged_bearers",
     "rs_group_create", "rs_group_create_checked", "rs_group_destroy", "rs_group_schedule_tti",
     "rs_group_get_slice_offset", "rs_group_set_slice_offset", "rs_group_launch_count", "rs_group_kernel_name",
@@ -121,6 +121,7 @@
     L.rs_last_error.restype = C.c_char_p
     L.rs_link_tables.argtypes = [C.POINTER(C.c_double)] * 4
     L.rs_link_tables_pinned.argtypes = [C.POINTER(C.c_double)] * 4
+    L.rs_link_y_table.argtypes = [C.c_int, C.c_int, C.c_int, C.POINTER(C.c_double)]
     L.rs_link_tables_compare.argtypes = [C.c_char_p, C.c_size_t]
     L.rs_ctx_jit_status.argtypes = [C.c_void_p, C.c_char_p, C.c_size_t]
     L.rs_jit_compiler_identity.restype = C.c_char_p
@@ -329,18 +330,26 @@
         (64 if counted else 0) | (128 if flows else 0) | (256 if run else 0)
 
 
+def _roomy_flags(roomy, group):
+    if roomy < 0 or roomy > 7 or (roomy & 6 and not roomy & 1):
+        raise ValueError("roomy is 0, or 1 plus any of 2 and 4")
+    if (roomy & 1) and group:
+        raise ValueError("roomy=1 excludes group=True: a group's kernels keep the plain carve")
+    return roomy << 9
+
+
 def jit_cache_file(n_slices, n_users, n_rbgs, rbg_size, threads=512, sched=RS_SCHED_MAXCELL, lean=False, streamed=False, group=False,
-                   resident=False, queued=False, counted=False, flows=False, run=False):
+                   resident=False, queued=False, counted=False, flows=False, run=False, roomy=0):
     buf = C.create_string_buffer(4096)
-    lib().rs_jit_cache_file(n_slices, n_users, n_rbgs, rbg_size, threads, sched, _jit_flags(lean, streamed, group, resident, queued, counted, flows, run),
+    lib().rs_jit_cache_file(n_slices, n_users, n_rbgs, rbg_size, threads, sched, _jit_flags(lean, streamed, group, resident, queued, counted, flows, run) | _roomy_flags(roomy, group),
                             buf, 4096)
     return buf.value.decode()
 
 
 def jit_cache_warm(n_slices, n_users, n_rbgs, rbg_size, threads=512, sched=RS_SCHED_MAXCELL, lean=False, streamed=False, group=False,
-                   resident=False, queued=False, counted=False, flows=False, run=False):
+                   resident=False, queued=False, counted=False, flows=False, run=False, roomy=0):
     buf = C.create_string_buffer(4096)
-    n = lib().rs_jit_cache_warm(n_slices, n_users, n_rbgs, rbg_size, threads, sched, _jit_flags(lean, streamed, group, resident, queued, counted, flows, run),
+    n = lib().rs_jit_cache_warm(n_slices, n_users, n_rbgs, rbg_size, threads, sched, _jit_flags(lean, streamed, group, resident, queued, counted, flows, run) | _roomy_flags(roomy, group),
                                 buf, 4096)
     if n < 0:
         raise RadioSaberError(n, buf.value.decode(errors="replace"))
@@ -397,6 +406,12 @@
     out = [np.zeros(16, np.float64) for _ in range(4)]
     _check((lib().rs_link_tables_pinned if pinned else lib().rs_link_tables)(*[_p(a, C.c_double) for a in out]))
     return dict(zip(("eff", "kbps", "eesm_e", "eesm_x"), out))
+
+
+def link_y_table(n_rbgs, rbg_size, pinned=True):
+    y = np.zeros((n_rbgs + 1, 14), np.float64)
+    _check(lib().rs_link_y_table(2 if pinned else 1, n_rbgs, rbg_size, _p(y, C.c_double)))
+    return y
 
 
 def link_tables_compare():
@@ -1121,8 +1136,8 @@
     def jit_status(self):
         if not getattr(self, "_h", None):
             raise RadioSaberError(-4, "jit_status() of a closed batch")
-        buf = C.create_string_buffer(512)
-        rc = lib().rs_batch_jit_status(self._h, buf, 512)
+        buf = C.create_string_buffer(768)
+        rc = lib().rs_batch_jit_status(self._h, buf, 768)
         return rc, buf.value.decode(errors="replace")
 
     def slice_bytes(self):
diff --git a/radiosaber_amd/csrc/rs_api.cpp b/radiosaber_amd/csrc/rs_api.cpp
--- a/radiosaber_amd/csrc/rs_api.cpp
+++ b/radiosaber_amd/csrc/rs_api.cpp
@@ -1,6 +1,7 @@
 #include <hip/hip_runtime_api.h>
 
 #include <atomic>
+#include <cfloat>
 #include <chrono>
 #include <cmath>
 #include <cstdarg>
@@ -232,6 +233,36 @@
   }
   for (int k = 2; k <= 13; k++)
     if (!(eesm_x[k] < eesm_x[k - 1])) return fail(RS_ERR_INVALID, "EESM thresholds not decreasing at %d", k);
+  return RS_OK;
+}
+
+static double la_y_largest(double n, double x, bool zero) {
+  auto holds = [&](double s) { const double q = s / n; return zero ? q == 0 : q <= x; };
+  uint64_t lo = 0, hi = to_bits(DBL_MAX);
+  while (hi - lo > 1) {
+    const uint64_t mid = lo + (hi - lo) / 2;
+    if (holds(from_bits(mid))) lo = mid; else hi = mid;
+  }
+  if (holds(from_bits(hi))) lo = hi;
+  return from_bits(lo);
+}
+static void la_y_fill(const double eesm_x[16], int R, int G, double* y) {
+  for (int k = 0; k < RS_LA_Y_COLS; k++) y[k] = 0;
+  for (int r = 1; r <= R; r++) {
+    const double n = (double)(r * G);
+    for (int k = 1; k <= 13; k++) y[(size_t)r * RS_LA_Y_COLS + k - 1] = la_y_largest(n, eesm_x[k], false);
+    y[(size_t)r * RS_LA_Y_COLS + 13] = la_y_largest(n, 0, true);
+  }
+}
+
+int rs_link_y_table(int link_tables, int n_rbgs, int rbg_size, double* y) {
+  if (!y) return fail(RS_ERR_INVALID, "null argument");
+  if (n_rbgs < 1 || n_rbgs > RS_MAX_RBGS || rbg_size < 1 || rbg_size > 8) return fail(RS_ERR_INVALID, "n_rbgs %d / rbg_size %d out of range", n_rbgs, rbg_size);
+  if (link_tables < RS_LINK_DEFAULT || link_tables > RS_LINK_PINNED_GLIBC_2_35) return fail(RS_ERR_INVALID, "link_tables %d is not an RS_LINK_* value", link_tables);
+  double eff[16], kbps[16], e[16], x[16];
+  const int rc = link_tables == RS_LINK_HOST_LIBM ? rs_link_tables(eff, kbps, e, x) : rs_link_tables_pinned(eff, kbps, e, x);
+  if (rc) return rc;
+  la_y_fill(x, n_rbgs, rbg_size, y);
   return RS_OK;
 }
 
@@ -256,6 +287,7 @@
   int32_t *d_eps = nullptr, *d_psi = nullptr;
   uint8_t* d_user_slice = nullptr;
   int32_t* d_tbs_eff = nullptr;
+  int roomy = 0;
   double* d_avg = nullptr;
   int32_t* d_tx = nullptr;
   int64_t *d_cumb = nullptr, *d_cumr = nullptr;
@@ -447,8 +479,14 @@
     std::vector<int32_t> te16((size_t)(b->R + 1) * 16, 0);
     for (int n = 0; n <= b->R; n++)
       for (int c = 0; c < 16; c++) te16[(size_t)n * 16 + c] = te[(size_t)n * 27 + t.itbs_of_cqi[c]];
-    HIP_TRY(hipMalloc(&b->d_tbs_eff, 4 * te16.size()));
+    std::vector<double> y;
+    if (b->roomy & 1) {
+      y.resize((size_t)(b->R + 1) * RS_LA_Y_COLS);
+      la_y_fill(t.eesm_x, b->R, b->G, y.data());
+    }
+    HIP_TRY(hipMalloc(&b->d_tbs_eff, 4 * te16.size() + 8 * y.size()));
     HIP_TRY(hipMemcpy(b->d_tbs_eff, te16.data(), 4 * te16.size(), hipMemcpyHostToDevice));
+    if (!y.empty()) HIP_TRY(hipMemcpy((char*)b->d_tbs_eff + 4 * te16.size(), y.data(), 8 * y.size(), hipMemcpyHostToDevice));
   }
   if (b->gen_exp) {
     std::vector<double> gn((size_t)S * 16, 0.0);
@@ -513,6 +551,20 @@
   return RS_OK;
 }
 
+int roomy_choice(const rs_batch* b) {
+  if (!b->jit_wanted || b->direct) return 0;
+  int steps = 3;
+  if (const char* e = getenv("RS_ROOMY_STEPS")) steps = atoi(e) & 3;
+  const char* const e = getenv("RS_ROOMY");
+  hipDeviceProp_t prop;
+  int cus = 256;
+  if (hipGetDeviceProperties(&prop, b->cfg.cell.device) == hipSuccess && prop.multiProcessorCount > 0) cus = prop.multiProcessorCount;
+  const RsCarve plain = rs_carve(b->S, b->U, b->R, b->sched, b->threads, 0, slice_window(b), RS_NVS_WHOLE_SLICE);
+  const bool on = !(e && atoi(e) == 0) && steps != 0 && b->n_cells <= 2 * cus && rs_roomy_fits(plain, b->S, b->R);
+  return on ? (1 | ((steps & 1) ? 0 : 2) | ((steps & 2) ? 0 : 4)) : 0;
+}
+int roomy_flags(const rs_batch* b) { return b->queues ? 0 : b->roomy << 9; }
+
 rs_batch* batch_new(const rs_batch_config* cfg, bool direct) {
   if (!cfg) { fail(RS_ERR_INVALID, "null config"); return nullptr; }
   if (validate(&cfg->cell, direct)) return nullptr;
@@ -573,11 +625,12 @@
   b->cfg.cell.slice_weight = nullptr; b->cfg.cell.algo_alpha = nullptr; b->cfg.cell.algo_beta = nullptr;
   b->cfg.cell.algo_epsilon = nullptr; b->cfg.cell.algo_psi = nullptr; b->cfg.cell.user_to_slice = nullptr;
   b->jit_wanted = want_jit && !direct;
+  b->roomy = roomy_choice(b);
   if (batch_alloc(b)) { rs_batch_destroy(b); return nullptr; }
   if (want_jit && !direct) {
     b->jit_wanted = true;
     b->jit = rs_jit_get(b->cfg.cell.device, b->S, b->U, b->R, b->G, b->threads, b->sched, 0, slice_window(b), b->jit_msg, sizeof b->jit_msg,
-                        b->cfg.cqi_refresh <= 4 ? 2 : 0);
+                        (b->cfg.cqi_refresh <= 4 ? 2 : 0) | roomy_flags(b));
     if (b->jit) snprintf(b->jit_msg, sizeof b->jit_msg, "%s", rs_jit_is_untuned(b->jit) ? "in use, built WITHOUT the -mllvm tuning options (hiprtc refused them): a few per cent slower" : "");
     else if (!b->jit_msg[0]) snprintf(b->jit_msg, sizeof b->jit_msg, "hiprtc build failed");
     if (!b->jit && b->threads > 512) {
@@ -611,7 +664,7 @@
     b->jit_lean_tried = true;
     char msg[512] = "";
     b->jit_lean = rs_jit_get(b->cfg.cell.device, b->S, b->U, b->R, b->G, b->threads, b->sched, b->queues ? b->qmode : 0, slice_window(b), msg,
-                             sizeof msg, (b->cfg.cqi_refresh <= 4 ? 2 : 0) | 4);
+                             sizeof msg, (b->cfg.cqi_refresh <= 4 ? 2 : 0) | 4 | roomy_flags(b));
     if (!b->jit_lean) snprintf(b->jit_msg, sizeof b->jit_msg, "lean build unavailable, the general build serves every launch (%.400s)", msg);
   }
   return b->jit_lean;
@@ -758,7 +811,7 @@
     char msg[512] = "";
     RsJitKernel* k = i == 0 ? k_default
                             : rs_jit_get(b->cfg.cell.device, b->S, b->U, b->R, b->G, b->threads, sched, 0, win, msg, sizeof msg,
-                                         (b->cfg.cqi_refresh <= 4 ? 2 : 0) | 4, cand[i].c_str());
+                                         (b->cfg.cqi_refresh <= 4 ? 2 : 0) | 4 | roomy_flags(b), cand[i].c_str());
     if (!k) { report += cand[i] + ": not built; "; continue; }
     b->jit_lean = k;
     float ms = 0;
@@ -1592,6 +1645,13 @@
   if (msg && msglen) snprintf(msg, msglen, "%s", b->jit_msg);
   if (b->jit_rejected) return -2;
   if (msg && msglen && b->jit && !b->jit_msg[0] && b->selfcheck_msg[0]) snprintf(msg, msglen, "%s", b->selfcheck_msg);
+  if (msg && msglen && b->jit) {
+    const size_t n = strlen(msg);
+    const int r = b->queues ? 0 : b->roomy;
+    if (n + 1 < msglen)
+      snprintf(msg + n, msglen - n, "%s%s LDS carve%s%s", n ? "; " : "", (r & 1) ? "roomy" : "plain", (r & 1) && (r & 2) ? ", no link-adaptation table" : "",
+               (r & 1) && (r & 4) ? ", no pristine sort records" : "");
+  }
   return b->jit ? 1 : (b->jit_wanted ? -1 : 0);
 }
 
diff --git a/radiosaber_amd/csrc/rs_device.h b/radiosaber_amd/csrc/rs_device.h
--- a/radiosaber_amd/csrc/rs_device.h
+++ b/radiosaber_amd/csrc/rs_device.h
@@ -58,6 +58,7 @@
   int Upad, n_seg, n_items, ept, nvs_seg;
   int off_avgk, off_rcp, off_tab, off_slice, off_tx, off_misc, off_tbs, off_elems, off_sorted, off_items,
       off_sortx, off_cqi, off_queue, off_qstate, q_lds, lds_bytes;
+  int off_lay, off_rec0;
 };
 constexpr int rs_round_up(int x, int a) { return (x + a - 1) / a * a; }
 constexpr int rs_upad_of(int U) {
@@ -149,6 +150,17 @@
   }
   return rs_carve_with(S, U, R, sched, threads, 0);
 }
+
+#define RS_LA_Y_COLS 14
+constexpr int rs_la_y_bytes(int R) { return rs_round_up(8 * RS_LA_Y_COLS * (R + 1), 16); }
+constexpr int rs_rec0_bytes(int S, int R) { return rs_round_up(4 * R * S, 16); }
+constexpr RsCarve rs_carve_roomy(RsCarve c, int S, int R) {
+  c.off_lay = rs_round_up(c.lds_bytes, 16);
+  c.off_rec0 = c.off_lay + rs_la_y_bytes(R);
+  c.lds_bytes = c.off_rec0 + rs_rec0_bytes(S, R);
+  return c;
+}
+constexpr bool rs_roomy_fits(const RsCarve& plain, int S, int R) { return 2 * rs_carve_roomy(plain, S, R).lds_bytes <= RS_LDS_LIMIT; }
 
 struct RsTables {
   double kbps[16];
diff --git a/radiosaber_amd/csrc/rs_jit.cpp b/radiosaber_amd/csrc/rs_jit.cpp
--- a/radiosaber_amd/csrc/rs_jit.cpp
+++ b/radiosaber_amd/csrc/rs_jit.cpp
@@ -43,8 +43,9 @@
 
 static std::vector<std::string> rs_jit_options(int S, int U, int R, int G, int NT, int sched, int qmode, int win, bool tuned, bool direct,
                                                bool streamed, bool lean, const char* variant = nullptr, bool group = false, bool resident = false,
-                                               bool queued = false, bool counted = false, bool flows = false, bool run = false) {
-  const RsCarve cv = rs_carve(S, U, R, sched, NT, qmode, win);
+                                               bool queued = false, bool counted = false, bool flows = false, bool run = false, int roomy = 0) {
+  const RsCarve plain = rs_carve(S, U, R, sched, NT, qmode, win);
+  const RsCarve cv = (roomy & 1) ? rs_carve_roomy(plain, S, R) : plain;
   std::vector<std::string> o = {"--offload-arch=gfx950", "-O3", "-std=c++17", "-ffp-contract=off", "-DRS_JIT_BUILD=1",
                                 "-DRS_JIT_S=" + std::to_string(S), "-DRS_JIT_U=" + std::to_string(U),
                                 "-DRS_JIT_R=" + std::to_string(R), "-DRS_JIT_G=" + std::to_string(G),
@@ -58,6 +59,11 @@
   if ((sched == 8 || sched == 101 || sched == 103) && !qmode && !direct && R <= 32 && (win > 32 || streamed)) o.push_back("-DRS_P3_BLOCK_TOP=8");
   if (streamed && !direct) o.push_back("-DRS_JIT_STREAMED=1");
   if (lean) o.push_back("-DRS_JIT_LEAN=1");
+  if (roomy & 1) {
+    o.push_back("-DRS_JIT_ROOMY=1");
+    if (roomy & 2) o.push_back("-DRS_NO_LA_TABLE");
+    if (roomy & 4) o.push_back("-DRS_NO_REC0");
+  }
   if (group) o.push_back("-DRS_JIT_GROUP=1");
   if (group && resident) o.push_back("-DRS_JIT_GROUP_RESIDENT=1");
   if (group && queued && !counted) o.push_back("-DRS_JIT_GROUP_QUEUED=1");
@@ -318,6 +324,10 @@
 
 static bool rs_jit_queued_sched(int sched) { return sched == 7 || sched == 8 || sched == 9 || sched == 101 || sched == 103; }
 static const char* rs_jit_group_flags_error(int flags, int sched) {
+  if ((flags & 512) != 0 && (flags & (1 | 8)) != 0)
+    return "flag value 512 (the roomy LDS carve) is a batch kernel's: it excludes 1 (the one-TTI form) and 8 (a group's build)";
+  if ((flags & (1024 | 2048)) != 0 && (flags & 512) == 0)
+    return "flag values 1024 and 2048 (the roomy carve without its table / its sort records) are valid only together with 512";
   if ((flags & 256) != 0 && ((flags & 8) == 0 || (flags & 16) == 0))
     return "flag value 256 (the run form) is valid only together with 8 (a group's build) and 16 (the resident form)";
   if ((flags & 256) != 0 && (flags & (32 | 64 | 128)) != 0)
@@ -347,7 +357,7 @@
     if (out && outlen) out[0] = 0;
     return 0;
   }
-  const std::vector<std::string> o = rs_jit_options(S, U, R, G, NT, sched, 0, equal_slices_window(S, U), true, (flags & 1) != 0 || (flags & 8) != 0, (flags & 2) != 0, (flags & 4) != 0, nullptr, (flags & 8) != 0, (flags & 16) != 0, (flags & 32) != 0, (flags & 64) != 0, (flags & 128) != 0, (flags & 256) != 0);
+  const std::vector<std::string> o = rs_jit_options(S, U, R, G, NT, sched, 0, equal_slices_window(S, U), true, (flags & 1) != 0 || (flags & 8) != 0, (flags & 2) != 0, (flags & 4) != 0, nullptr, (flags & 8) != 0, (flags & 16) != 0, (flags & 32) != 0, (flags & 64) != 0, (flags & 128) != 0, (flags & 256) != 0, (flags >> 9) & 7);
   const std::string file = cache_file_of(cache_key_text(o));
   if (out && outlen) snprintf(out, outlen, "%s", file.c_str());
   return (int)file.size();
@@ -359,7 +369,7 @@
     if (err && errlen) snprintf(err, errlen, "%s", why);
     return -1;
   }
-  const std::vector<char> code = rs_jit_code(rs_jit_options(S, U, R, G, NT, sched, 0, equal_slices_window(S, U), true, (flags & 1) != 0 || (flags & 8) != 0, (flags & 2) != 0, (flags & 4) != 0, nullptr, (flags & 8) != 0, (flags & 16) != 0, (flags & 32) != 0, (flags & 64) != 0, (flags & 128) != 0, (flags & 256) != 0), log);
+  const std::vector<char> code = rs_jit_code(rs_jit_options(S, U, R, G, NT, sched, 0, equal_slices_window(S, U), true, (flags & 1) != 0 || (flags & 8) != 0, (flags & 2) != 0, (flags & 4) != 0, nullptr, (flags & 8) != 0, (flags & 16) != 0, (flags & 32) != 0, (flags & 64) != 0, (flags & 128) != 0, (flags & 256) != 0, (flags >> 9) & 7), log);
   if (code.empty()) {
     if (err && errlen) snprintf(err, errlen, "%.*s", (int)errlen - 1, log.c_str());
     return -1;
@@ -474,6 +484,11 @@
   const bool run = (flags & 256) != 0;
   if (const char* why = rs_jit_group_flags_error(flags, sched)) {
     if (err && errlen) snprintf(err, errlen, "shape-specialised kernel unavailable (flags: %s)", why);
+    return nullptr;
+  }
+  const int roomy = (flags >> 9) & 7;
+  if ((roomy & 1) != 0 && qmode != 0) {
+    if (err && errlen) snprintf(err, errlen, "shape-specialised kernel unavailable (flags: value 512, the roomy LDS carve, excludes the queue model)");
     return nullptr;
   }
   const int direct = (flags & 1) | (group ? 1 : 0);
@@ -496,11 +511,11 @@
   }
   std::string log, file, key_text;
   bool untuned = false, from_cache = false, verified = false;
-  std::vector<char> code = rs_jit_code(rs_jit_options(S, U, R, G, NT, sched, qmode, win, true, direct != 0, streamed, lean, variant, group, resident, queued, counted, flows, run), log, &file, &key_text,
+  std::vector<char> code = rs_jit_code(rs_jit_options(S, U, R, G, NT, sched, qmode, win, true, direct != 0, streamed, lean, variant, group, resident, queued, counted, flows, run, roomy), log, &file, &key_text,
                                        &from_cache, &verified);
   if (code.empty() && !getenv("RS_JIT_NO_RETRY")) {
     std::string log2;
-    code = rs_jit_code(rs_jit_options(S, U, R, G, NT, sched, qmode, win, false, direct != 0, streamed, lean, variant, group, resident, queued, counted, flows, run), log2, &file, &key_text, &from_cache,
+    code = rs_jit_code(rs_jit_options(S, U, R, G, NT, sched, qmode, win, false, direct != 0, streamed, lean, variant, group, resident, queued, counted, flows, run, roomy), log2, &file, &key_text, &from_cache,
                        &verified);
     untuned = !code.empty();
   }
diff --git a/radiosaber_amd/csrc/rs_kernels.hip b/radiosaber_amd/csrc/rs_kernels.hip
--- a/radiosaber_amd/csrc/rs_kernels.hip
+++ b/radiosaber_amd/csrc/rs_kernels.hip
@@ -80,6 +80,13 @@
 #ifndef RS_JIT_CARVEQ
 #define RS_JIT_CARVEQ 0
 #endif
+#ifndef RS_JIT_ROOMY
+#define RS_JIT_ROOMY 0
+#endif
+constexpr RsCarve rs_jit_carve() {
+  const RsCarve c = rs_carve(RS_JIT_S, RS_JIT_U, RS_JIT_R, RS_JIT_SCHED, RS_JIT_NT, RS_JIT_CARVEQ, RS_JIT_WIN);
+  return RS_JIT_ROOMY ? rs_carve_roomy(c, RS_JIT_S, RS_JIT_R) : c;
+}
 
 template <int SCHED, int EPT, bool FIXED, bool DIRECT, bool QUEUE = false, bool GROUP = false>
 __device__ __forceinline__ void rs_cell_body(const RsLaunch& p, unsigned char* lds) {
@@ -116,7 +123,7 @@
   const int nt = FIXED ? RS_JIT_NT : (int)blockDim.x;
   const int lane = lane_id(), wave = wave_id(), nwaves = nt >> 6;
   const int S = FIXED ? RS_JIT_S : p.S, U = (FIXED && !DIRECT) ? RS_JIT_U : p.U, R = FIXED ? RS_JIT_R : p.R, G = FIXED ? RS_JIT_G : p.G;
-  constexpr RsCarve kCv = rs_carve(RS_JIT_S, RS_JIT_U, RS_JIT_R, RS_JIT_SCHED, RS_JIT_NT, RS_JIT_CARVEQ, RS_JIT_WIN);
+  constexpr RsCarve kCv = rs_jit_carve();
   struct Offs { int avgk, rcp, tab, slice, tx, misc, tbs, elems, sorted, items, sortx, cqi, queue, Upad, n_seg, n_items; };
   const Offs o = FIXED ? Offs{kCv.off_avgk, kCv.off_rcp, kCv.off_tab, kCv.off_slice, kCv.off_tx, kCv.off_misc, kCv.off_tbs,
                               kCv.off_elems, kCv.off_sorted, kCv.off_items, kCv.off_sortx, kCv.off_cqi, kCv.off_queue,
@@ -178,6 +185,14 @@
   int32_t* s_tbs = (int32_t*)(lds + o.tbs);
   uint8_t* s_cqi = lds + o.cqi;
   const int Upad = o.Upad;
+  constexpr bool kRoomy = FIXED && RS_JIT_ROOMY && !DIRECT && !QUEUE && !GROUP;
+#ifdef RS_NO_LA_TABLE
+  constexpr bool kLaTable = false;
+#else
+  constexpr bool kLaTable = kRoomy;
+#endif
+  const double* const s_lay = (const double*)(lds + kCv.off_lay);
+  uint32_t* const s_rec0 = (uint32_t*)(lds + kCv.off_rec0);
 
   const RsTables* tab = p.tab;
   RsCellScalars* scal = p.scal + cell;
@@ -247,6 +262,8 @@
     }
   }
   for (int i = tid; i < (R + 1) * 16; i += nt) s_tbs[i] = p.tbs_eff[i];
+  if constexpr (kLaTable)
+    for (int i = tid; i < (R + 1) * RS_LA_Y_COLS; i += nt) ((double*)(lds + kCv.off_lay))[i] = ((const double*)(p.tbs_eff + (R + 1) * 16))[i];
   if (!grid_from_image)
     for (int i = tid; i < (R * Upad) >> 2; i += nt) ((uint32_t*)s_cqi)[i] = 0;
   for (int i = tid; i < Upad + 16 * S; i += nt) s_rcp32[i] = 0.0f;
@@ -634,6 +651,9 @@
 #ifndef RS_JIT_GROUP_RUN
 #define RS_JIT_GROUP_RUN 0
 #endif
+#if RS_JIT_ROOMY && (RS_JIT_GROUP || RS_JIT_DIRECT || RS_JIT_CARVEQ)
+#error "RS_JIT_ROOMY: the roomy carve is a batch kernel's without the queue model; drop-in and group builds keep the plain carve"
+#endif
 #if RS_JIT_GROUP
 #if RS_JIT_GROUP_RESIDENT && RS_JIT_GROUP_QUEUED
 #error "RS_JIT_GROUP_RESIDENT and RS_JIT_GROUP_QUEUED exclude each other"
@@ -704,7 +724,7 @@
   p.gate = nullptr; p.exact_scan = 0; p.gen_exp = 0; p.gen_num = nullptr; p.log_upper = nullptr; p.synthetic = 0;
   p.trace = nullptr; p.trace_prb = nullptr; p.epochs_prb = nullptr; p.log_keys = nullptr;
 #endif
-  constexpr RsCarve kCv = rs_carve(RS_JIT_S, RS_JIT_U, RS_JIT_R, RS_JIT_SCHED, RS_JIT_NT, RS_JIT_CARVEQ, RS_JIT_WIN);
+  constexpr RsCarve kCv = rs_jit_carve();
   __shared__ __align__(16) unsigned char lds[kCv.lds_bytes];
   constexpr int kEpt = (RS_JIT_SCHED != 9 && RS_JIT_SCHED != 10) ? 0 : (kCv.ept <= 4 ? kCv.ept : 0);
   rs_cell_body<RS_JIT_SCHED, kEpt, true, RS_JIT_DIRECT != 0, (RS_JIT_CARVEQ >= 2)>(p, lds);
diff --git a/radiosaber_amd/csrc/rs_phase_p3.inc b/radiosaber_amd/csrc/rs_phase_p3.inc
--- a/radiosaber_amd/csrc/rs_phase_p3.inc
+++ b/radiosaber_amd/csrc/rs_phase_p3.inc
@@ -8,6 +8,11 @@
       nvs_runs = idiv_small(nvs_hi - nvs_first + nvs_seg - 1, nvs_seg);
     }
     const int n_items = nvs_split ? R * nvs_runs : o.n_items;
+#ifdef RS_NO_REC0
+    constexpr bool kRec0 = false;
+#else
+    constexpr bool kRec0 = kRoomy && kHoldSched && SCHED == 9;
+#endif
     auto scan_item = [&](int it, uint16_t* bu_out, uint32_t* rec_out, auto blk_tag) -> bool {
       bool held = false;
       float top1 = 0.0f, top2 = 0.0f;
@@ -171,6 +176,7 @@
           rec_out[sg * R + r] = ((uint32_t)bkey << 16) | ((uint32_t)r << 8) | (uint32_t)sg;
         } else if (kTransport) {
           rec_out[r * S + sg] = ((uint32_t)bkey << 16) | ((uint32_t)r << 8) | (uint32_t)sg;
+          if constexpr (kRec0) s_rec0[r * S + sg] = ((uint32_t)bkey << 16) | ((uint32_t)r << 8) | (uint32_t)sg;
         } else if (SCHED == 1 || nvs_split) {
           s_best_metric[it] = best;
         }
@@ -349,6 +355,7 @@
               }
               cur_bu[it] = (uint16_t)ul;
               if (SCHED != 9) cur_rec[r * S + sg] = ((uint32_t)key << 16) | ((uint32_t)r << 8) | (uint32_t)sg;
+              else if constexpr (kRec0) s_rec0[r * S + sg] = ((uint32_t)key << 16) | ((uint32_t)r << 8) | (uint32_t)sg;
               const int kk = FIXED ? it / (RS_JIT_NT / 64) : idiv_small(it, nwaves);
               unsigned long long* const word = &hold_bits[(kk >> 6) * nwaves + wave];
               if (held) atomicOr(word, 1ull << (kk & 63));
diff --git a/radiosaber_amd/csrc/rs_phase_p4.inc b/radiosaber_amd/csrc/rs_phase_p4.inc
--- a/radiosaber_amd/csrc/rs_phase_p4.inc
+++ b/radiosaber_amd/csrc/rs_phase_p4.inc
@@ -6,6 +6,9 @@
         RS_SETPRIO(1);
         if constexpr (kHoldSched) {
           if (!hold_full) {
+            if constexpr (kRec0) {
+              for (int x = tid; x < N; x += nt) s_elems[x] = s_rec0[x];
+            } else
             for (int x = tid; x < N; x += nt) {
               const int r = FIXED ? x / RS_JIT_S : idiv_small(x, S), sg = x - r * S;
               const int bu = cur_bu[sg * R + r];
diff --git a/radiosaber_amd/csrc/rs_phase_p5.inc b/radiosaber_amd/csrc/rs_phase_p5.inc
--- a/radiosaber_amd/csrc/rs_phase_p5.inc
+++ b/radiosaber_amd/csrc/rs_phase_p5.inc
@@ -142,6 +142,16 @@
           if (lane == 0) __hip_atomic_store(&m->grid_free, tti + 1, __ATOMIC_RELAXED, __HIP_MEMORY_SCOPE_WORKGROUP);
         }
         if (leader) {
+          if constexpr (kLaTable) {
+            const double* const yr = s_lay + (FIXED ? nprb / RS_JIT_G : nprb / G) * RS_LA_Y_COLS;
+            double yv[RS_LA_Y_COLS];
+#pragma unroll
+            for (int k = 0; k < RS_LA_Y_COLS; ++k) yv[k] = yr[k];
+            int cnt = 1;
+#pragma unroll
+            for (int k = 0; k < 13; ++k) cnt += (sum <= yv[k]) ? 1 : 0;
+            fcqi = sum <= yv[13] ? 15 : cnt;
+          } else {
           const double x = sum / (double)nprb;
           if (x == 0) {
             fcqi = 15;
@@ -149,6 +159,7 @@
             fcqi = 1;
 #pragma unroll
             for (int k = 1; k <= 13; ++k) fcqi += (x <= xthr_k[k - 1]) ? 1 : 0;
+          }
           }
           RS_P5STAMP(4);
           mcs = m->mcs_of_cqi[fcqi];
```

Result: no change. 43.91 million (median of 6 runs) (+0.7%).
